# QiminWu/mceik

Measured on AMD Instinct MI355X. Metric: MCMC proposals/sec (FSM eikonal + likelihood), 128³ grid, 1/2/4/8 MI355X, higher is better.
Workload: dtype f32

## Files before the change

mceik_amd/csrc/capi.hip:

```cpp
#include <hip/hip_runtime.h>
#include <float.h>
#include <math.h>
#include <stdint.h>
#include <stdio.h>
#include <stdlib.h>
#include <string.h>
#include <unistd.h>

#include <algorithm>
#include <vector>

#include "../../include/mceik.h"
#include "fsm_common.h"
#include "mcmc_common.h"
#include "fsm_single.h"
#include "rccl_rt.h"
#include "posterior.h"
#include "temper.h"

hipError_t fsm_launch(const FsmLaunch &L, int is_double, int nwaves, hipStream_t st);
hipError_t fsm_zero_words(unsigned *p, int n, hipStream_t st);
int fsm_occupancy(const FsmLaunch &L, int is_double);
size_t fsm_launch_lds_bytes(const FsmLaunch &L, int is_double);
int fsm_launch_kind(const FsmLaunch &L, int is_double);
const char *fsm_launch_name(const FsmLaunch &L, int is_double);
hipError_t fsm_to_brick_f64(const double *src, void *dst, int dst_double, const FsmLaunch &L, int nfield, hipStream_t st);
hipError_t fsm_from_brick_f64(const void *src, int src_double, double *dst, const FsmLaunch &L, int nfield, hipStream_t st);
hipError_t fsm_from_brick_f32(const float *src, float *dst, const FsmLaunch &L, int nfield, hipStream_t st);
hipError_t fsm_to_brick_f32(const float *src, float *dst, const FsmLaunch &L, int nfield, hipStream_t st);
hipError_t mcmc_propose(const McmcDev &D, uint64_t step, hipStream_t st);
hipError_t mcmc_init_loglik(const McmcDev &D, hipStream_t st);
hipError_t mcmc_accept(const McmcDev &D, int keep_slot, hipStream_t st);
hipError_t mcmc_lpt_order(const unsigned long long *clk, int nsolve, int *order, hipStream_t st);
hipError_t l2_gridsearch_f32(int ldgrd, int ngrd, int nev, int iwantOT, float t0use, const int *ev_ptr,
                             const int *obs_row, const float *tc, const float *wt, const float *xnorm,
                             const float *test, float *t0, float *objfn, int negate, hipStream_t st);
size_t relocate_lds_bytes(int nrows, int nobs, int nev);
hipError_t relocate_lds(int ldgrd, int ngrd, int nrows, int nev, int nobs, int iwantOT, float t0use,
                        const int *ev_ptr, const int *obs_row, const float *tc, const float *wt, const float *xnorm,
                        const float *test, float *t0, float *objfn, int negate, hipStream_t st);
hipError_t gridsearch_f90(int is_double, int ldgrd, int ngrd, int nuse, int iwantOT, const int *row,
                          const void *tob, const void *w0, const void *wl, const void *test, void *logpdf,
                          hipStream_t st);
hipError_t l2_gridsearch(int ldgrd, int ngrd, int nuse, int iwantOT, double t0use, const int *use,
                         const double *tc, const double *wt, double xnorm, const double *test,
                         double *t0, double *objfn, hipStream_t st);

#define HIPCHK(x)                                                                      \
    do {                                                                               \
        hipError_t e_ = (x);                                                           \
        if (e_ != hipSuccess) {                                                        \
            fprintf(stderr, "mceik_hip: %s failed: %s (%s:%d)\n", #x,                  \
                    hipGetErrorString(e_), __FILE__, __LINE__);                        \
            return -1;                                                                 \
        }                                                                              \
    } while (0)

static double conv_threshold(double tol, int is_double)
{
    double tolr = is_double ? tol : (double)(float)tol;
    if (!(tolr > 0.0)) return HUGE_VAL;
    int p = is_double ? 53 : 24;
    int k = (int)ceil(log2(tolr)) + p;
    while (ldexp(1.0, k - p) < tolr) k++;
    while (ldexp(1.0, k - 1 - p) >= tolr) k--;
    double T = ldexp(1.0, k);
    double big = is_double ? DBL_MAX : (double)FLT_MAX;
    return T > big ? HUGE_VAL : T;
}

static void fill_launch(FsmLaunch &L, const mceik_fsm_batch *b)
{
    memset(&L, 0, sizeof(L));
    L.nx = b->nx; L.ny = b->ny; L.nz = b->nz;
    fsm_geometry(&L, b->precision == 64 ? 8 : 4);
    L.maxit = b->maxit; L.max_sweeps = b->max_sweeps;
    L.tol = b->tol; L.h = b->h; L.x0 = b->x0; L.y0 = b->y0; L.z0 = b->z0;
    int is_double = b->precision == 64;
    double T = conv_threshold(b->tol, is_double);
    L.conv_thresh = is_double ? (T == HUGE_VAL ? DBL_MAX : T) : (T == HUGE_VAL ? (double)FLT_MAX : T);
    L.nsolve = b->nmodel * b->nstat; L.nstat = b->nstat; L.nsrc = b->nsrc;
    L.src = b->src;
    L.slow_mode = b->slow_mode;
    L.nrx = b->nrx > 0 ? b->nrx : 1; L.nry = b->nry > 0 ? b->nry : 1; L.nrz = b->nrz > 0 ? b->nrz : 1;
    L.ncx = mceik_div_up(L.nx, L.nrx); L.ncy = mceik_div_up(L.ny, L.nry); L.ncz = mceik_div_up(L.nz, L.nrz);
    L.magic_rx = ((1u << 20) + L.nrx - 1) / L.nrx;
    L.magic_ry = ((1u << 20) + L.nry - 1) / L.nry;
    L.magic_rz = ((1u << 20) + L.nrz - 1) / L.nrz;
    L.ev_node = b->ev_node; L.nev = b->nev; L.ttab = b->ttab; L.ev_frac = b->ev_frac;
    L.model_phase = b->slow_mode == 1 ? b->model_phase : nullptr;
    L.skip = b->skip;
    L.solve_count = b->solve_count;
    L.nphase = b->nphase > 0 ? b->nphase : 1;
    {
        auto span = [](int a, int e, int nr) { return e / nr - a / nr + 1; };
        int mx = 0, my = 0, mz = 0;
        for (int t = 0; t < L.ntx; t++) {
            int v = span(t * 8, t * 8 + 7 < L.nx - 1 ? t * 8 + 7 : L.nx - 1, L.nrx); mx = v > mx ? v : mx;
        }
        for (int t = 0; t < L.nty; t++) {
            int v = span(t * 8, t * 8 + 7 < L.ny - 1 ? t * 8 + 7 : L.ny - 1, L.nry); my = v > my ? v : my;
        }
        for (int t = 0; t < L.nzk; t++) {
            int a = t * L.kb * 8, e = a + L.kb * 8 - 1 < L.nz - 1 ? a + L.kb * 8 - 1 : L.nz - 1;
            int v = span(a, e, L.nrz); mz = v > mz ? v : mz;
        }
        L.ccb = mx * my * mz;
        L.cell_cache = b->slow_mode == 1 && L.ccb <= MCEIK_CC_MAX && L.nx < 4096 && L.ny < 4096 && L.nz < 4096;
        if (!L.cell_cache) L.ccb = 0;
    }
    L.fast_sqrt = b->fast_sqrt;
    L.niter = b->niter; L.ierr = b->ierr;
    L.iter_total = b->iter_total;
    L.visit_stats = b->visit_stats;
    L.solve_order = b->solve_order;
    L.solve_clock = b->solve_clock;
    L.max_waves = b->max_waves;
    L.traffic = b->traffic;
    L.step_z = b->step_z;
}

static int g_device_cus = 0;

static int device_cus()
{
    if (g_device_cus == 0) {
        int dev = 0;
        hipDeviceProp_t p;
        if (hipGetDevice(&dev) == hipSuccess && hipGetDeviceProperties(&p, dev) == hipSuccess)
            g_device_cus = p.multiProcessorCount;
        else
            g_device_cus = 256;
    }
    return g_device_cus;
}

static size_t ws_budget_bytes()
{
    static size_t budget = 0;
    if (budget == 0) {
        const char *e = getenv("MCEIK_FSM_WS_GB");
        double gb = e ? atof(e) : 0.0;
        if (gb > 0.0) {
            budget = (size_t)(gb * 1073741824.0);
        } else {
            size_t fr = 0, tot = 0;
            const size_t margin = (size_t)8 << 30;
            if (hipMemGetInfo(&fr, &tot) == hipSuccess && tot) {
                budget = tot / 5 * 4;
                const size_t avail = fr > 2 * margin ? fr - margin : fr / 2;
                if (avail < budget) budget = avail;
            } else {
                budget = (size_t)96 << 30;
            }
        }
    }
    return budget;
}

static int batch_waves(const FsmLaunch &L, int is_double)
{
    int per_cu = fsm_occupancy(L, is_double);
    if (per_cu < 1) per_cu = 1;
    static const int env_cap = [] { const char *e = getenv("MCEIK_WAVES_PER_CU"); return e ? atoi(e) : 0; }();
    if (env_cap > 0 && env_cap < per_cu) per_cu = env_cap;
    long w = (long)per_cu * device_cus();
    if (L.max_waves > 0 && w > L.max_waves) w = L.max_waves;
    if (w > L.nsolve) w = L.nsolve;
    static const bool report = getenv("MCEIK_LAUNCH_REPORT") != nullptr;
    if (report)
        fprintf(stderr, "mceik fsm launch: %d-z steps, %d waves/CU (occupancy), %ld resident waves, %zu B LDS per wave\n",
                fsm_launch_kind(L, is_double), per_cu, w, fsm_launch_lds_bytes(L, is_double));
    return (int)(w < 1 ? 1 : w);
}

static int fsm_batch_waves_uncapped(const mceik_fsm_batch *b)
{
    FsmLaunch L;
    fill_launch(L, b);
    return batch_waves(L, b->precision == 64);
}

struct WsLayout {
    size_t counter, slow, u, u0, zf, total;
    int nwaves;
};

static WsLayout ws_layout(const mceik_fsm_batch *b)
{
    FsmLaunch L;
    fill_launch(L, b);
    int is_double = b->precision == 64;
    size_t es = is_double ? 8 : 4;
    WsLayout w;
    w.nwaves = batch_waves(L, is_double);
    const size_t zfw = fsm_launch_kind(L, is_double) == 16 ? zf_bytes(L, es) : 0;
    {
        const size_t per_wave = 2 * L.field_elems * es + zfw;
        const long cap = (long)(ws_budget_bytes() / (per_wave ? per_wave : 1));
        if (cap >= 1 && w.nwaves > cap) w.nwaves = (int)cap;
    }
    w.counter = 0;
    w.slow = 1024;
    size_t slow_bytes = b->slow_mode == 0 ? (size_t)b->nmodel * L.field_elems * es : 0;
    w.u = w.slow + ((slow_bytes + 255) & ~(size_t)255);
    size_t nu = b->u_out ? (size_t)L.nsolve : (size_t)w.nwaves;
    w.u0 = w.u + nu * L.field_elems * es;
    w.zf = w.u0 + (size_t)w.nwaves * L.field_elems * es;
    w.total = w.zf + (size_t)w.nwaves * zfw;
    return w;
}

extern "C" size_t mceik_fsm_workspace_bytes(const mceik_fsm_batch *b)
{
    return ws_layout(b).total;
}

extern "C" int mceik_fsm_step_z(const mceik_fsm_batch *b)
{
    if (!b) return 0;
    FsmLaunch L;
    fill_launch(L, b);
    return fsm_launch_kind(L, b->precision == 64);
}

extern "C" const char *mceik_fsm_kernel_name(const mceik_fsm_batch *b)
{
    if (!b) return "";
    FsmLaunch L;
    fill_launch(L, b);
    return fsm_launch_name(L, b->precision == 64);
}

extern "C" size_t mceik_fsm_lds_bytes(const mceik_fsm_batch *b)
{
    if (!b) return 0;
    FsmLaunch L;
    fill_launch(L, b);
    return fsm_launch_lds_bytes(L, b->precision == 64);
}

extern "C" double mceik_fsm_bytes_per_node_sweep(const mceik_fsm_batch *b)
{
    double es = b->precision == 64 ? 8.0 : 4.0;
    double s = b->slow_mode == 0 ? es : 4.0 / ((double)b->nrx * b->nry * b->nrz);
    return 2.0 * es + s / (b->nstat > 0 ? b->nstat : 1);
}

#define MCEIK_MC_CHUNK 64
struct McmcExt {
    const void *dev;
    unsigned *sync;
    unsigned spin_limit;
    int step0, nsteps, nburn, keepk, maxs, nkept0;
};

static int fsm_batch_solve_impl(const mceik_fsm_batch *b, void *workspace, size_t workspace_bytes, void *stream,
                                const McmcExt *ext);

extern "C" int mceik_fsm_batch_solve(const mceik_fsm_batch *b, void *workspace, size_t workspace_bytes,
                                     void *stream)
{
    return fsm_batch_solve_impl(b, workspace, workspace_bytes, stream, nullptr);
}

static int fsm_batch_solve_impl(const mceik_fsm_batch *b, void *workspace, size_t workspace_bytes, void *stream,
                                const McmcExt *ext)
{
    if (!b || b->nx < 2 || b->ny < 2 || b->nz < 2 || b->nx > 4096 || b->ny > 4096 || b->nz > 4096 ||
        b->nsrc < 1 ||
        b->nmodel < 1 || b->nstat < 1 || !(b->precision == 32 || b->precision == 64)) {
        fprintf(stderr, "mceik_fsm_batch_solve: invalid batch description\n");
        return 1;
    }
    if (b->slow_mode == 1 && b->precision != 32 && b->precision != 64) return 1;
    WsLayout w = ws_layout(b);
    {
        FsmLaunch G;
        fill_launch(G, b);
        if (G.field_elems * (b->precision == 64 ? 8 : 4) >= (size_t)1 << 31) {
            fprintf(stderr, "mceik_fsm_batch_solve: one travel-time field must stay below 2 GiB\n");
            return 1;
        }
        if (fsm_launch_lds_bytes(G, b->precision == 64) > MCEIK_MAX_LDS) {
            fprintf(stderr, "mceik_fsm_batch_solve: %d x %d x %d z-blocks exceed the LDS block tables\n", G.ntx, G.nty,
                    G.nzk);
            return 1;
        }
        const bool held = fsm_launch_kind(G, b->precision == 64) == 16 || fsm_compact_layout(G, 8);
        const int infl = fsm_launch_kind(G, b->precision == 64) == 16 ? fsm16_geo(G).infl : G.infl;
        if (held && hold_clock_bound(G.nblocks, infl) >= 65536) {
            fprintf(stderr, "mceik_fsm_batch_solve: %d z-blocks overflow the held stream's 16-bit clocks\n", G.nblocks);
            return 1;
        }
    }
    if (!workspace || workspace_bytes < w.total) {
        fprintf(stderr, "mceik_fsm_batch_solve: workspace too small (%zu < %zu)\n", workspace_bytes, w.total);
        return 1;
    }
    if (b->skip && b->u_out) {
        fprintf(stderr, "mceik_fsm_batch_solve: skip and u_out cannot be combined (a skipped solve has no field)\n");
        return 1;
    }
    hipStream_t st = (hipStream_t)stream;
    int is_double = b->precision == 64;
    FsmLaunch L;
    fill_launch(L, b);
    char *ws = (char *)workspace;
    L.counter = (unsigned *)(ws + w.counter);
    HIPCHK(fsm_zero_words(L.counter, 256, st));
    if (b->slow_mode == 0) {
        void *sb = ws + w.slow;
        if (is_double)
            HIPCHK(fsm_to_brick_f64((const double *)b->slow, sb, 1, L, b->nmodel, st));
        else
            HIPCHK(fsm_to_brick_f32((const float *)b->slow, (float *)sb, L, b->nmodel, st));
        L.slow = sb;
    } else {
        L.slow = b->slow;
    }
    L.u = ws + w.u;
    L.u0 = ws + w.u0;
    L.zf = ws + w.zf;
    L.slot_per_solve = b->u_out ? 1 : 0;
    if (ext) {
        if (is_double || fsm_launch_kind(L, 0) != 16 || b->solve_order || b->u_out) return 1;
        L.mc_dev = ext->dev;
        L.mc_sync = ext->sync;
        L.mc_spin_limit = ext->spin_limit;
        L.mc_step0 = ext->step0; L.mc_nsteps = ext->nsteps;
        L.mc_nburn = ext->nburn; L.mc_keepk = ext->keepk; L.mc_maxs = ext->maxs; L.mc_nkept0 = ext->nkept0;
        HIPCHK(fsm_zero_words(ext->sync, MC_SYNC_WORDS(L.nsolve / L.nstat) - 1, st));
    }
    HIPCHK(fsm_launch(L, is_double, w.nwaves, st));
    if (b->u_out) {
        if (is_double) HIPCHK(fsm_from_brick_f64(L.u, 1, (double *)b->u_out, L, L.nsolve, st));
        else HIPCHK(fsm_from_brick_f32((const float *)L.u, (float *)b->u_out, L, L.nsolve, st));
    }
    return 0;
}

static bool is_device_ptr(const void *p)
{
    hipPointerAttribute_t a;
    if (!p || hipPointerGetAttributes(&a, p) != hipSuccess) {
        (void)hipGetLastError();
        return false;
    }
    return a.type == hipMemoryTypeDevice;
}

extern "C" int eikonal3d_batch_solve(int nmodels, int nstations, int nx, int ny, int nz, double h, double x0,
                                     double y0, double z0, int maxit, double tol, const double *src,
                                     const float *slow, float *u, int *niter, int *ierr)
{
    if (nmodels < 1 || nstations < 1 || !src || !slow || !u) return 1;
    const size_t n = (size_t)nx * ny * nz, nsolve = (size_t)nmodels * nstations;
    mceik_fsm_batch b;
    memset(&b, 0, sizeof(b));
    b.nx = nx; b.ny = ny; b.nz = nz; b.h = h; b.x0 = x0; b.y0 = y0; b.z0 = z0;
    b.maxit = maxit; b.tol = tol; b.precision = 32;
    b.nmodel = nmodels; b.nstat = nstations; b.nsrc = 1; b.slow_mode = 0; b.max_sweeps = -1;
    std::vector<void *> tmp;
    auto stage = [&](const void *p, size_t bytes, bool in) -> void * {
        if (is_device_ptr(p)) return const_cast<void *>(p);
        void *d = nullptr;
        if (hipMalloc(&d, bytes) != hipSuccess) return nullptr;
        tmp.push_back(d);
        if (in && hipMemcpy(d, p, bytes, hipMemcpyHostToDevice) != hipSuccess) return nullptr;
        return d;
    };
    int rc = 0;
    void *d_src = stage(src, (size_t)nstations * 4 * sizeof(double), true);
    void *d_slow = stage(slow, (size_t)nmodels * n * sizeof(float), true);
    void *d_u = stage(u, nsolve * n * sizeof(float), false);
    void *d_it = niter ? stage(niter, nsolve * sizeof(int), false) : nullptr;
    void *d_ie = ierr ? stage(ierr, nsolve * sizeof(int), false) : nullptr;
    void *ws = nullptr;
    if (!d_src || !d_slow || !d_u || (niter && !d_it) || (ierr && !d_ie)) rc = -1;
    if (!rc) {
        b.src = (const double *)d_src; b.slow = d_slow; b.u_out = d_u;
        b.niter = (int *)d_it; b.ierr = (int *)d_ie;
        const size_t wsb = mceik_fsm_workspace_bytes(&b);
        if (hipMalloc(&ws, wsb) != hipSuccess) rc = -1;
        else rc = mceik_fsm_batch_solve(&b, ws, wsb, nullptr);
        if (!rc && hipDeviceSynchronize() != hipSuccess) rc = -1;
    }
    if (!rc && d_u != u) rc = hipMemcpy(u, d_u, nsolve * n * sizeof(float), hipMemcpyDeviceToHost) != hipSuccess;
    if (!rc && niter && d_it != niter) rc = hipMemcpy(niter, d_it, nsolve * sizeof(int), hipMemcpyDeviceToHost) != hipSuccess;
    if (!rc && ierr && d_ie != ierr) rc = hipMemcpy(ierr, d_ie, nsolve * sizeof(int), hipMemcpyDeviceToHost) != hipSuccess;
    if (ws) hipFree(ws);
    for (void *p : tmp) hipFree(p);
    return rc;
}

extern "C" int mceik_memcpy(void *dst, const void *src, size_t bytes, int kind)
{
    hipMemcpyKind k = kind == 0 ? hipMemcpyHostToDevice : kind == 1 ? hipMemcpyDeviceToHost : hipMemcpyDeviceToDevice;
    HIPCHK(hipMemcpy(dst, src, bytes, k));
    return 0;
}

struct SingleState {
    int init;
    int nx, ny, nz, maxit_cap, nsrc_cap;
    int is_double;
    SingleLaunch L;
    void *mem;
    double *dense, *src;
    int *ierr_bc;
    int nwaves;
    int bcfail;
    hipStream_t st;
    int iverb, maxit;
    double x0, y0, z0, h, tol;
    BlockDecomp D;
    double *snap;
    unsigned *d_count;
};
static SingleState g_single[3];

static void single_free(SingleState &S)
{
    if (S.snap) hipFree(S.snap);
    if (S.d_count) hipFree(S.d_count);
    if (S.mem) hipFree(S.mem);
    if (S.st) hipStreamDestroy(S.st);
    const SingleState keep = S;
    memset(&S, 0, sizeof(S));
    S.init = keep.init;
    S.iverb = keep.iverb; S.maxit = keep.maxit;
    S.x0 = keep.x0; S.y0 = keep.y0; S.z0 = keep.z0; S.h = keep.h; S.tol = keep.tol;
    S.D = keep.D;
}

static int blocks_buffers(SingleState &S)
{
    const size_t np = (size_t)S.L.nxp * S.L.nyp * S.L.nzp;
    if (!S.snap && hipMalloc(&S.snap, np * 8) != hipSuccess) { S.snap = nullptr; return 1; }
    if (!S.d_count && hipMalloc(&S.d_count, 16) != hipSuccess) { S.d_count = nullptr; return 1; }
    return 0;
}

static int single_alloc(SingleState &S, int is_double, int nx, int ny, int nz, int maxit, int nsrc)
{
    if (S.mem && S.is_double == is_double && S.nx == nx && S.ny == ny && S.nz == nz && maxit <= S.maxit_cap &&
        nsrc <= S.nsrc_cap)
        return 0;
    const int keep = S.init;
    single_free(S);
    S.init = keep;
    if (nx < 1 || ny < 1 || nz < 1 || (long)nx * ny * nz >= (1L << 31)) return 1;
    SingleLaunch &L = S.L;
    L.nx = nx; L.ny = ny; L.nz = nz;
    L.gx = nx; L.gy = ny; L.gz = nz;
    L.nbx = mceik_div_up(nx, 8); L.nby = mceik_div_up(ny, 8); L.nbz = mceik_div_up(nz, 8);
    if (L.nbx > 1024 || L.nby > 1024 || L.nbz > 1024) return 1;
    L.nxp = 8 * L.nbx; L.nyp = 8 * L.nby; L.nzp = 8 * L.nbz;
    L.nb = L.nbx * L.nby * L.nbz;
    if ((size_t)L.nxp * L.nyp * L.nzp * (is_double ? 8 : 4) >= ((size_t)1 << 31)) return 1;
    const int mcap = maxit > 0 ? maxit : 1, scap = nsrc > 0 ? nsrc : 1;
    const size_t es = is_double ? 8 : 4, np = (size_t)L.nxp * L.nyp * L.nzp, n = (size_t)nx * ny * nz;
    auto al = [](size_t v) { return (v + 255) & ~(size_t)255; };
    size_t off[12], o = 0;
    off[0] = o; o += al(np * es);
    off[1] = o; o += al(np * es);
    off[2] = o; o += al(np * es);
    off[3] = o; o += al(np);
    off[4] = o; o += al((size_t)L.nb * 4);
    off[5] = o; o += al((size_t)L.nb * 4);
    off[6] = o; o += al((size_t)(32 + mcap) * 4);
    off[7] = o; o += al((size_t)mcap * 8);
    off[8] = o; o += al((size_t)mcap * 4);
    off[9] = o; o += al(n * 8);
    off[10] = o; o += al((size_t)scap * 32);
    off[11] = o; o += al(16);
    if (hipMalloc(&S.mem, o) != hipSuccess) { S.mem = nullptr; return 1; }
    char *m = (char *)S.mem;
    L.u = m + off[0]; L.u0 = m + off[1]; L.slow = m + off[2]; L.bc = (unsigned char *)(m + off[3]);
    L.border = (const int *)(m + off[4]); L.done = (unsigned *)(m + off[5]); L.ctl = (unsigned *)(m + off[6]);
    L.arrive = (unsigned long long *)(m + off[7]); L.ierr_it = (int *)(m + off[8]);
    S.dense = (double *)(m + off[9]); S.src = (double *)(m + off[10]); S.ierr_bc = (int *)(m + off[11]);
    L.bcerr = S.ierr_bc;
    std::vector<int> ord;
    ord.reserve(L.nb);
    for (int lev = 0; lev <= L.nbx + L.nby + L.nbz - 3; lev++)
        for (int bz = 0; bz < L.nbz; bz++)
            for (int by = 0; by < L.nby; by++) {
                const int bx = lev - bz - by;
                if (bx >= 0 && bx < L.nbx) ord.push_back(bx | (by << 10) | (bz << 20));
            }
    if ((int)ord.size() != L.nb ||
        hipMemcpy((void *)L.border, ord.data(), ord.size() * 4, hipMemcpyHostToDevice) != hipSuccess ||
        hipStreamCreateWithFlags(&S.st, hipStreamNonBlocking) != hipSuccess) {
        single_free(S);
        return 1;
    }
    static const int wpc = [] { const char *e = getenv("MCEIK_SINGLE_WAVES_PER_CU"); return e ? atoi(e) : 2; }();
    int occ = fsm_single_occupancy(is_double);
    S.nwaves = device_cus() * std::max(1, std::min(wpc, occ));
    S.is_double = is_double; S.nx = nx; S.ny = ny; S.nz = nz; S.maxit_cap = mcap; S.nsrc_cap = scap;
    return 0;
}

static int single_solve(SingleState &S, int maxit, int nsrc, double tol, double h, double x0, double y0, double z0,
                        const double *ts, const double *xs, const double *ys, const double *zs, const double *slow,
                        double *u, int *niter_out)
{
    SingleLaunch &L = S.L;
    const size_t n = (size_t)L.nx * L.ny * L.nz;
// ... 1861 lines not shown
```

mceik_amd/csrc/fsm16_kernel.hip:

```cpp
#include <hip/hip_runtime.h>
#include <float.h>
#include <stdint.h>

#include "fsm_common.h"
#include "fsm_device.h"
#include "fsm_hold.h"
#include "fsm_update.h"
#include "mcmc_device.h"

namespace {

__device__ __forceinline__ uint32_t zoff16(int zb)
{
    const uint32_t u = (uint32_t)zb;
    return ((u >> 1) << 13) | ((u & 1u) << 6);
}

#ifdef MCEIK_PHASECLK
#undef TRAF
#undef TRAFU
#define TRAF(S, k, pred, bytes) do { } while (0)
#define TRAFU(S, k, bytes) do { } while (0)
#define PCLK(k)                                                                                         \
    do {                                                                                                \
        const unsigned long long t_ = __builtin_readcyclecounter();                                     \
        if (threadIdx.x == 0) S.scratch[8 + (k)] += (int)(t_ - pclk_t);                                 \
        pclk_t = t_;                                                                                    \
    } while (0)
#else
#define PCLK(k) do { } while (0)
#endif

struct Smem16 {
    int *box;
    float *cc;
    unsigned short *order;
    unsigned short *lastproc;
    unsigned short *lastchg;
    int *ring_e, *ring_b;
    unsigned *ring_base;
    unsigned *fmask;
    int *scratch;
    float *xr;
    unsigned *meta;
    unsigned char *fz;
    unsigned *vbits, *cbits;
};
template <bool FIXED>
__device__ __forceinline__ Smem16 smem16_bind(const FsmLaunch &L, unsigned char *base)
{
    size_t off[MCEIK_SMEM16_ARRAYS];
    if (FIXED) {
        off[8] = F16_CINFO; off[7] = F16_XR; off[1] = F16_CC; off[5] = F16_RING; off[6] = F16_SCRATCH;
        off[3] = F16_LASTPROC; off[4] = F16_LASTCHG; off[2] = F16_ORDER;
        off[9] = F16_ORDER + mceik_align16((size_t)L.ntiles * 2);
        off[10] = off[9] + mceik_align16((size_t)L.ntiles);
        off[0] = off[10] + f16_bitmap_bytes(L);
    } else {
        fsm16_smem_layout(L, off);
    }
    const int nr = fsm16_geo(L).nr;
    Smem16 S;
    S.box = reinterpret_cast<int *>(base + off[0]);
    S.cc = reinterpret_cast<float *>(base + off[1]);
    S.order = reinterpret_cast<unsigned short *>(base + off[2]);
    S.lastproc = reinterpret_cast<unsigned short *>(base + off[3]);
    S.lastchg = reinterpret_cast<unsigned short *>(base + off[4]);
    S.ring_e = reinterpret_cast<int *>(base + off[5]);
    S.ring_b = S.ring_e + (FIXED ? F16_NR : nr);
    S.ring_base = reinterpret_cast<unsigned *>(S.ring_b + (FIXED ? F16_NR : nr));
    S.fmask = S.ring_base + (FIXED ? F16_NR : nr);
    S.fz = base + off[9];
    S.vbits = reinterpret_cast<unsigned *>(base + off[10]);
    S.cbits = S.vbits + (L.nblocks + 31) / 32;
    S.scratch = reinterpret_cast<int *>(base + off[6]);
    S.xr = reinterpret_cast<float *>(base + off[7]);
    S.meta = reinterpret_cast<unsigned *>(base + off[8]);
    return S;
}

#define XROW16(arr, q, row) (((arr) * 4 + (q)) * MCEIK_X16Q + (row) * 4)
typedef float f4v16 __attribute__((ext_vector_type(4)));
__device__ __forceinline__ void lds_w4(float *p, float a, float b, float c, float d)
{
    *reinterpret_cast<f4v16 *>(p) = f4v16{a, b, c, d};
}
__device__ __forceinline__ void lds_r4(const float *p, float &a, float &b, float &c, float &d)
{
    const f4v16 v = *reinterpret_cast<const f4v16 *>(p);
    a = v.x; b = v.y; c = v.z; d = v.w;
}
__device__ __forceinline__ void store_row16(float *x, int arr, int lane, const float (&v)[16])
{
#pragma unroll
    for (int q = 0; q < 4; q++) lds_w4(x + XROW16(arr, q, lane), v[4 * q], v[4 * q + 1], v[4 * q + 2], v[4 * q + 3]);
}
__device__ __forceinline__ void load_row16(const float *x, int arr, int row, float (&v)[16])
{
#pragma unroll
    for (int q = 0; q < 4; q++) lds_r4(x + XROW16(arr, q, row), v[4 * q], v[4 * q + 1], v[4 * q + 2], v[4 * q + 3]);
}
__device__ __forceinline__ void load_half16(const float *x, int arr, int row, int h, float (&v)[8])
{
    lds_r4(x + XROW16(arr, 2 * h, row), v[0], v[1], v[2], v[3]);
    lds_r4(x + XROW16(arr, 2 * h + 1, row), v[4], v[5], v[6], v[7]);
}
__device__ __forceinline__ void halo_stage16(float *x, int lane, const float (&v)[8])
{
    const int j = lane >> 1, h = lane & 1;
    const int arr = (j >> 3) & 1, row = 64 + ((j >> 4) << 3) + (j & 7);
    lds_w4(x + XROW16(arr, 2 * h, row), v[0], v[1], v[2], v[3]);
    lds_w4(x + XROW16(arr, 2 * h + 1, row), v[4], v[5], v[6], v[7]);
}

#define NPASS16 4
#define W1_ZD (1u << 24)

__device__ __forceinline__ void seg_issue(Rsrc r, uint32_t seg, float (&a)[16])
{
    const bool odd = threadIdx.x & 1;
    const uint32_t segp = dpp_swap_pair(seg);
    float t[4];
    bload4(r, odd ? segp + 16u : seg, t);
    a[0] = t[0]; a[1] = t[1]; a[2] = t[2]; a[3] = t[3];
    bload4(r, odd ? segp + 48u : seg + 32u, t);
    a[4] = t[0]; a[5] = t[1]; a[6] = t[2]; a[7] = t[3];
    bload4(r, odd ? seg + 16u : segp, t);
    a[8] = t[0]; a[9] = t[1]; a[10] = t[2]; a[11] = t[3];
    bload4(r, odd ? seg + 48u : segp + 32u, t);
    a[12] = t[0]; a[13] = t[1]; a[14] = t[2]; a[15] = t[3];
}
#define XQE MCEIK_X16Q
__device__ __forceinline__ int pair_row(int arr, int lane)
{
    return (lane & 1) ? XROW16(arr, 1, lane - 1) : XROW16(arr, 0, lane);
}
__device__ __forceinline__ void raw_write(float *x, int pb, const float (&a)[16])
{
    lds_w4(x + pb, a[0], a[1], a[2], a[3]);
    lds_w4(x + pb + 2 * XQE, a[4], a[5], a[6], a[7]);
    lds_w4(x + pb + 4, a[8], a[9], a[10], a[11]);
    lds_w4(x + pb + 2 * XQE + 4, a[12], a[13], a[14], a[15]);
}
__device__ __forceinline__ void raw_read(const float *x, int pb, float (&a)[16])
{
    lds_r4(x + pb, a[0], a[1], a[2], a[3]);
    lds_r4(x + pb + 2 * XQE, a[4], a[5], a[6], a[7]);
    lds_r4(x + pb + 4, a[8], a[9], a[10], a[11]);
    lds_r4(x + pb + 2 * XQE + 4, a[12], a[13], a[14], a[15]);
}
template <int P>
struct Par16 {
    static constexpr int value = P;
};

struct LineLd {
    float a[8];
    int rowl, rowo;
};
__device__ __forceinline__ void line_issue(Rsrc r, uint32_t seg, bool isl, LineLd &q, float (&h)[8])
{
    const int lane = threadIdx.x, par = lane & 1;
    const bool islp = dpp_swap_pair((unsigned)isl) != 0u;
    const uint32_t segp = dpp_swap_pair(seg);
    const uint32_t sl = isl ? seg : (islp ? segp : OOB);
    const uint32_t o = (uint32_t)par * 16u;
    float t[4];
    bload4(r, sl + o, t);
    q.a[0] = t[0]; q.a[1] = t[1]; q.a[2] = t[2]; q.a[3] = t[3];
    bload4(r, sl + o + 32u, t);
    q.a[4] = t[0]; q.a[5] = t[1]; q.a[6] = t[2]; q.a[7] = t[3];
    const uint32_t sh = sl ^ 64u;
    bload4(r, sh + o, t);
    h[0] = t[0]; h[1] = t[1]; h[2] = t[2]; h[3] = t[3];
    bload4(r, sh + o + 32u, t);
    h[4] = t[0]; h[5] = t[1]; h[6] = t[2]; h[7] = t[3];
    q.rowl = isl ? lane : (lane ^ 1);
    q.rowo = lane ^ (q.rowl == lane ? 1 : 0);
}
__device__ __forceinline__ void line_write(float *x, const LineLd &q, const float (&hp)[8])
{
    const int par = threadIdx.x & 1;
    lds_w4(x + XROW16(1, par, q.rowl), q.a[0], q.a[1], q.a[2], q.a[3]);
    lds_w4(x + XROW16(1, par + 2, q.rowl), q.a[4], q.a[5], q.a[6], q.a[7]);
    lds_w4(x + XROW16(1, par, q.rowo), hp[0], hp[1], hp[2], hp[3]);
    lds_w4(x + XROW16(1, par + 2, q.rowo), hp[4], hp[5], hp[6], hp[7]);
}

__device__ __forceinline__ void raw_store(Rsrc r, uint32_t seg, bool chg, const float (&t)[16])
{
    const bool odd = threadIdx.x & 1;
    const uint32_t own = chg ? seg : OOB;
    const uint32_t oth = dpp_swap_pair(own);
    const uint32_t o = odd ? 16u : 0u;
    const uint32_t b01 = (odd ? oth : own) + o, b23 = (odd ? own : oth) + o;
    bstore4(r, b01, t[0], t[1], t[2], t[3]);
    bstore4(r, b01 + 32u, t[4], t[5], t[6], t[7]);
    bstore4(r, b23, t[8], t[9], t[10], t[11]);
    bstore4(r, b23 + 32u, t[12], t[13], t[14], t[15]);
}
__device__ __forceinline__ void store16_plain(Rsrc r, uint32_t off, const float (&v)[16])
{
#pragma unroll
    for (int q = 0; q < 4; q++) bstore4(r, off + 16u * q, v[4 * q], v[4 * q + 1], v[4 * q + 2], v[4 * q + 3]);
}

__device__ __forceinline__ void bload4h(Rsrc r, uint32_t off, float (&v)[4])
{
    f4v a = __builtin_bit_cast(f4v, __builtin_amdgcn_raw_buffer_load_b128(r, off, 0, 0));
    v[0] = a.x; v[1] = a.y; v[2] = a.z; v[3] = a.w;
}
struct BInfo16 {
    uint32_t seg;
    uint32_t zh;
    uint32_t lseg;
    uint32_t w1, w2, w3;
    __device__ __forceinline__ int fl() const { return (int)(w1 & 0xfffu); }
    __device__ __forceinline__ int zb() const { return (int)((w1 >> 12) & 0xffu); }
    __device__ __forceinline__ int ri() const { return (int)((w1 >> 20) & 0xfu); }
    __device__ __forceinline__ int ccb() const { return (int)(w2 << 16) >> 16; }
    __device__ __forceinline__ int clk() const { return (int)(w2 >> 16); }
    __device__ __forceinline__ int bid() const { return (int)(w3 & 0xffffu); }
    __device__ __forceinline__ int bcm() const { return (int)(w3 >> 16); }
};
template <bool RZ>
__device__ __forceinline__ BInfo16 brick_info16(const FsmLaunch &L, const Fsm16Geo &g, int kb, const Smem16 &S,
                                                const Pos &p, int nstream, int lx, int ly, const BcBoxes &bc,
                                                unsigned meta, uint32_t col)
{
    BInfo16 b;
    const int tz = ci_tz(meta);
    const int zb = tz * kb + (RZ ? kb - 1 - p.zbs : p.zbs);
    const bool valid = pos_valid(p, nstream) && (meta & C_BLK) && zb < g.nzb;
    b.seg = valid ? col + zoff16(zb) : OOB;
    b.lseg = pos_valid(p, nstream) && (meta & C_BLK) && (zb & ~1) < g.nzb ? col + zoff16(zb) : OOB;
    const int zu = RZ ? zb * 16 + 16 : zb * 16 - 1;
    b.zh = (valid && (meta & C_ZH) && p.zbs == 0) ? col + zoff16(zu >> 4) + (uint32_t)(zu & 15) * 4u : OOB;
    int fl = valid ? (int)((meta & 0x7f) | F_VALID) : 0;
    if (zb == (RZ ? g.nzb - 1 : 0)) fl |= F_FIRST;
    if (zb == (RZ ? 0 : g.nzb - 1)) fl |= F_LAST;
    const bool zd = valid && p.zbs == kb - 1 && !(fl & F_LAST);
    if (b.zh != OOB) b.zh = zf_boundary<float, RZ>(L, S.ring_b[p.ri], false, lx, ly);
    if (zd) b.zh = zf_boundary<float, RZ>(L, S.ring_b[p.ri], true, lx, ly);
    if ((meta & C_ZH) && p.zbs == 0) fl |= F_ZH;
    bool slow = (fl & C_PART) || ((fl & C_00) && zb == 0) || (valid && zb * 16 + 16 > L.nz);
    unsigned bcm = 0;
    if (__any(fl & C_BC)) {
        const int e = S.ring_e[p.ri];
        const int x = (e & 0xfff) * 8 + lx, y = ((e >> 12) & 0xfff) * 8 + ly;
        unsigned m = 0;
        if (fl & C_BC) {
            for (int k = 0; k < bc.n; k++) {
                const int *q = bc.box + 6 * k;
                if (x >= q[0] && x <= q[1] && y >= q[2] && y <= q[3]) {
                    int lo = q[4] - zb * 16, hi = q[5] - zb * 16;
                    lo = lo < 0 ? 0 : lo; hi = hi > 15 ? 15 : hi;
                    if (lo <= hi) m |= ((2u << hi) - (1u << lo));
                }
            }
        }
        bcm = m;
        slow |= m != 0;
    }
    if (slow) fl |= F_SLOW;
    const int ccb = ci_ccb(meta) + zb * 4;
    b.w1 = (uint32_t)fl | ((uint32_t)(valid ? zb : 0) << 12) | ((uint32_t)p.ri << 20) | (zd ? W1_ZD : 0u);
    b.w2 = ((uint32_t)ccb & 0xffffu) | ((uint32_t)p.sp << 16);
    b.w3 = ((uint32_t)S.ring_b[p.ri] & 0xffffu) | (bcm << 16);
    return b;
}
template <bool RZ>
__device__ __forceinline__ uint32_t halo_offset16(const Fsm16Geo &g, int kb, const Pos &pe, int nstream, int half,
                                                  unsigned meta, uint32_t col, unsigned hbit, uint32_t hdelta)
{
    const int zb = ci_tz(meta) * kb + (RZ ? kb - 1 - pe.zbs : pe.zbs);
    const bool valid = pos_valid(pe, nstream) && (meta & C_BLK) && zb < g.nzb;
    const uint32_t base = col + ((meta & hbit) ? 0u : hdelta);
    return valid ? base + zoff16(zb) + (uint32_t)half * 32u : OOB;
}

#define LW_G(p) (9 + 5 * (p))
#define LW_CCB 19
template <bool RZ>
__device__ __forceinline__ unsigned lean_word(const FsmLaunch &L, const Fsm16Geo &g, const ColTile &ct, int tz, int ri,
                                              int u0flag, int zh)
{
    int cz0, nczb;
    block_zcells(L, L.kb, tz, cz0, nczb);
    const int m = ct.fl | C_BLK | (u0flag ? C_U0 : 0) | (zh ? C_ZH : 0);
    const int zb0 = 2 * tz + (RZ ? 1 : 0);
    unsigned w = (unsigned)m & 0x1ffu;
#pragma unroll
    for (int p = 0; p < 2; p++) {
        const int zb = RZ ? zb0 - p : zb0 + p;
        unsigned gp = zb < g.nzb ? 16u : 0u;
        if (zb == (RZ ? g.nzb - 1 : 0)) gp |= 1u;
        if (zb == (RZ ? 0 : g.nzb - 1)) gp |= 2u;
        if ((m & C_PART) || ((m & C_00) && zb == 0) || zb * 16 + 16 > L.nz) gp |= 4u;
        if (p == 0 && (m & C_ZH)) gp |= 8u;
        w |= gp << LW_G(p);
    }
    const int ccb0 = ri * L.ccb + ct.cl * nczb - cz0 + zb0 * 4;
    return w | ((unsigned)ccb0 << LW_CCB);
}
template <bool RZ>
__device__ __forceinline__ BInfo16 brick_info_lean(const FsmLaunch &L, const Smem16 &S, const Pos &p, int nstream,
                                                   int lx, int ly, const BcBoxes &bc, unsigned w, uint32_t base)
{
    BInfo16 b;
    const int ph = p.zbs;
    const unsigned gp = (w >> (ph ? LW_G(1) : LW_G(0))) & 31u;
    const bool pv = pos_valid(p, nstream);
    const bool valid = pv && (gp & 16u);
    const uint32_t off = base + ((uint32_t)(ph ^ (RZ ? 1 : 0)) << 6);
    b.seg = valid ? off : OOB;
    b.lseg = pv && (w & ((16u << LW_G(0)) | (16u << LW_G(1)))) ? off : OOB;
    b.zh = valid && (gp & 8u) ? off + (RZ ? 8192u - 64u : 124u - 8192u) : OOB;
    const bool zd = valid && ph == 1 && !(gp & 2u);
    if (b.zh != OOB) b.zh = zf_boundary<float, RZ>(L, S.ring_b[p.ri], false, lx, ly);
    if (zd) b.zh = zf_boundary<float, RZ>(L, S.ring_b[p.ri], true, lx, ly);
    int fl = valid ? (int)((w & 0x7fu) | F_VALID | ((gp & 15u) << 8)) : 0;
    unsigned bcm = 0;
    if (__any(fl & C_BC)) {
        const int e = S.ring_e[p.ri];
        const int zb = 2 * ((e >> 24) & 0xff) + (RZ ? 1 - ph : ph);
        const int x = (e & 0xfff) * 8 + lx, y = ((e >> 12) & 0xfff) * 8 + ly;
        if (fl & C_BC) {
            for (int k = 0; k < bc.n; k++) {
                const int *q = bc.box + 6 * k;
                if (x >= q[0] && x <= q[1] && y >= q[2] && y <= q[3]) {
                    int lo = q[4] - zb * 16, hi = q[5] - zb * 16;
                    lo = lo < 0 ? 0 : lo; hi = hi > 15 ? 15 : hi;
                    if (lo <= hi) bcm |= ((2u << hi) - (1u << lo));
                }
            }
        }
        if (bcm) fl |= F_SLOW;
    }
    const int ccb = (int)(w >> LW_CCB) + (RZ ? -4 * ph : 4 * ph);
    b.w1 = (uint32_t)fl | ((uint32_t)ph << 12) | ((uint32_t)p.ri << 20) | (zd ? W1_ZD : 0u);
    b.w2 = ((uint32_t)ccb & 0xffffu) | ((uint32_t)p.sp << 16);
    b.w3 = ((uint32_t)S.ring_b[p.ri] & 0xffffu) | (bcm << 16);
    return b;
}
template <bool RZ>
__device__ __forceinline__ uint32_t halo_offset_lean(const Pos &pe, int nstream, int half, unsigned me, uint32_t base,
                                                     unsigned hbit, uint32_t hdelta)
{
    const int ph = pe.zbs;
    const bool valid = pos_valid(pe, nstream) && ((me >> (ph ? LW_G(1) : LW_G(0))) & 16u);
    const uint32_t o = base + ((me & hbit) ? 0u : hdelta) + ((uint32_t)(ph ^ (RZ ? 1 : 0)) << 6) + (uint32_t)half * 32u;
    return valid ? o : OOB;
}
template <bool RZ>
__device__ __forceinline__ uint32_t halo_line_lean(const Pos &pe, int nstream, unsigned me, uint32_t base,
                                                   unsigned hbit, uint32_t hdelta)
{
    const bool valid = pos_valid(pe, nstream) && (me & ((16u << LW_G(0)) | (16u << LW_G(1))));
    return valid ? base + ((me & hbit) ? 0u : hdelta) : OOB;
}
__device__ __forceinline__ unsigned dpp_swap_quad_half(unsigned v)
{
    return (unsigned)__builtin_amdgcn_mov_dpp((int)v, 0x4E, 0xf, 0xf, false);
}
template <bool RZ, bool LEAN>
__device__ __forceinline__ BInfo16 brick_info_any(const FsmLaunch &L, const Fsm16Geo &g, int kb, const Smem16 &S,
                                                  const Pos &p, int nstream, int lx, int ly, const BcBoxes &bc,
                                                  unsigned meta, uint32_t col)
{
    if (LEAN) return brick_info_lean<RZ>(L, S, p, nstream, lx, ly, bc, meta, col);
    return brick_info16<RZ>(L, g, kb, S, p, nstream, lx, ly, bc, meta, col);
}
template <bool RZ, bool LEAN>
__device__ __forceinline__ uint32_t halo_offset_any(const Fsm16Geo &g, int kb, const Pos &pe, int nstream, int half,
                                                    unsigned meta, uint32_t col, unsigned hbit, uint32_t hdelta)
{
    if (LEAN) return halo_offset_lean<RZ>(pe, nstream, half, meta, col, hbit, hdelta);
    return halo_offset16<RZ>(g, kb, pe, nstream, half, meta, col, hbit, hdelta);
}

__device__ __forceinline__ void build_order16(const FsmLaunch &L, unsigned short *order)
{
    for (int id = threadIdx.x; id < L.ntiles; id += 64) {
        const int txs = id % L.ntx, tys = id / L.ntx, dg = txs + tys;
        int rank = 0;
        for (int e = 0; e < dg; e++)
            rank += min(e, L.nty - 1) - max(0, e - L.ntx + 1) + 1;
        rank += tys - max(0, dg - L.ntx + 1);
        order[rank] = (unsigned short)(txs | (tys << 8));
    }
}


__device__ __forceinline__ HoldLds<unsigned short> hold_lds16(const Smem16 &S)
{
    HoldLds<unsigned short> H;
    H.order = S.order; H.fz = S.fz; H.lastproc = S.lastproc; H.need = S.lastchg; H.fmask = S.fmask;
    H.ring_e = S.ring_e; H.vbits = S.vbits; H.cbits = S.cbits;
    return H;
}


template <bool RZ, bool LEAN>
__device__ __forceinline__ void admit16(const FsmLaunch &L, const Fsm16Geo &g, const Smem16 &S, const BcBoxes &bc,
                                        int entry, int zh, int u0flag, int ri, int C, int lx, int ly, int lxs,
                                        int lys, int rx, int ry, ColTile &ct)
{
    unsigned meta = 0;
    int bid = 0, nbv = 0;
    uint32_t base = 0;
    if (entry >= 0) {
        const int tz = (entry >> 24) & 0xff, tx = entry & 0xfff, ty = (entry >> 12) & 0xfff;
        bid = tz * L.ntiles + tx + ty * L.ntx;
        nbv = min(L.kb, L.nzb - tz * L.kb);
        if ((entry & 0xffffff) != ct.tile) column_tile<float>(L, bc, entry, lx, ly, lxs, lys, rx, ry, ct);
        meta = LEAN ? lean_word<RZ>(L, g, ct, tz, ri, u0flag, zh) : column_word(L, L.kb, ct, tz, ri, u0flag, zh);
        base = (uint32_t)(ty * L.ntx + tx) * tile_bytes<float>(L) + (LEAN ? (uint32_t)tz << 13 : 0u);
    }
    const int nact = L.visit_stats && entry >= 0 ? __builtin_popcountll(__ballot(ct.fl & C_ACT)) : 0;
    asm volatile("" ::: "memory");
    S.meta[ri * 64 + threadIdx.x] = meta;
    if (threadIdx.x == 0) {
        if (entry >= 0) {
            S.lastproc[bid] = (unsigned short)C;
            S.vbits[bid >> 5] |= 1u << (bid & 31);
            if (L.visit_stats) {
                S.scratch[0] += nbv;
                S.scratch[1] += nbv * nact;
            }
        }
        S.ring_e[ri] = entry;
        S.ring_b[ri] = bid;
        S.ring_base[ri] = base;
    }
    asm volatile("" ::: "memory");
}


template <bool RZ, bool GENERIC, bool LEAN, bool NC = true>
__device__ __forceinline__ void brick16(const FsmLaunch &L, const Smem16 &S, const BInfo16 &b0, float (&v)[16],
                                        float zprev0, float znext, int lx, int ly, int rx, int ry, bool &changed,
                                        bool &nc, int &ierr_last, bool &c0, bool &c15)
{
    const int lane = threadIdx.x;
    const float T = (float)L.conv_thresh;
    const int fl = b0.fl();
    bool xp = true, xn = true, yp = true, yn = true, act = true;
    int zbg = 0;
    if (GENERIC) {
        const int e = S.ring_e[b0.ri()];
        zbg = LEAN ? 2 * ((e >> 24) & 0xff) + (RZ ? 1 - b0.zb() : b0.zb()) : b0.zb();
        const int x = (e & 0xfff) * 8 + lx, y = ((e >> 12) & 0xfff) * 8 + ly;
        const bool xlo = x > 0, xhi = x < L.nx - 1, ylo = y > 0, yhi = y < L.ny - 1;
        xp = rx ? xhi : xlo; xn = rx ? xlo : xhi; yp = ry ? yhi : ylo; yn = ry ? ylo : yhi;
        act = (fl & C_ACT) != 0;
    }
    const bool first = (fl & F_FIRST) != 0, last = (fl & F_LAST) != 0;
    const int lxs = lane & 7, lys = lane >> 3;
    const int rxm = lxs > 0 ? lane - 1 : 64 + lys, rym = lys > 0 ? lane - 8 : 72 + lxs;
    const int rxp = lxs < 7 ? lane + 1 : 64 + lys, ryp = lys < 7 ? lane + 8 : 72 + lxs;
    float fc = 0.f, ffc = 0.f, ff2c = 0.f, ff3c = 0.f;
#pragma unroll
    for (int hh = 0; hh < NPASS16; hh++) {
        constexpr int PZ = 16 / NPASS16;
        const int h = RZ ? NPASS16 - 1 - hh : hh;
        float xm[PZ], xq[PZ], ym[PZ], yq[PZ];
        lds_r4(S.xr + XROW16(0, h, rxm), xm[0], xm[1], xm[2], xm[3]);
        lds_r4(S.xr + XROW16(0, h, rym), ym[0], ym[1], ym[2], ym[3]);
        lds_r4(S.xr + XROW16(1, h, rxp), xq[0], xq[1], xq[2], xq[3]);
        lds_r4(S.xr + XROW16(1, h, ryp), yq[0], yq[1], yq[2], yq[3]);
#pragma unroll
        for (int jj = 0; jj < PZ; jj++) {
            const int j = hh * PZ + jj;
            const int pj = RZ ? 15 - j : j;
            const int ph = pj % PZ;
            const int pprev = RZ ? pj + 1 : pj - 1, pnext = RZ ? pj - 1 : pj + 1;
            const float self = v[pj];
            if (!GENERIC) {
                if ((j & 3) == 0) {
                    fc = S.cc[b0.ccb() + (pj >> 2)];
                    ffc = fc * fc;
                    ff2c = ffc + ffc;
                    ff3c = 3.0f * ffc;
                }
            }
            float xup = xm[ph], xdn = xq[ph], yup = ym[ph], ydn = yq[ph];
            float zup, zdn;
            if (GENERIC) {
                xup = xp ? xup : self; xdn = xn ? xdn : self; yup = yp ? yup : self; ydn = yn ? ydn : self;
                const int zabs = zbg * 16 + pj;
                const bool zp_ex = RZ ? (zabs < L.nz - 1) : (zabs > 0);
                const bool zn_ex = RZ ? (zabs > 0) : (zabs < L.nz - 1);
                zup = zp_ex ? (j > 0 ? v[pprev] : zprev0) : self;
                zdn = zn_ex ? (j < 15 ? v[pnext] : znext) : self;
            } else {
                zup = j > 0 ? v[pprev] : (first ? self : zprev0);
                zdn = j < 15 ? v[pnext] : (last ? self : znext);
            }
            const float ux = fmin_(xup, xdn), uy = fmin_(yup, ydn), uz = fmin_(zup, zdn);
            float nv;
            if (GENERIC) {
                const int zabs = zbg * 16 + pj;
                const int zc_ = zabs < L.nz ? zabs : L.nz - 1;
                const float f = S.cc[b0.ccb() - zbg * 4 + (zc_ >> 2)];
                int e;
                const float ub = godunov_bl<true>(ux, uy, uz, f, e);
                const bool upd = act && zabs < L.nz && !((b0.bcm() >> pj) & 1);
                nv = upd ? fmin_(self, ub) : self;
                if ((fl & C_00) && zabs == 0) ierr_last = upd ? e : 0;
            } else {
                nv = fmin_(self, godunov_v<true>(ux, uy, uz, fc, ffc, ff2c, ff3c));
            }
            const bool dec = nv < self;
            if (NC) nc |= dec && self >= T;
            changed |= dec;
            if (pj == 0) c0 = dec;
            if (pj == 15) c15 = dec;
            v[pj] = nv;
        }
    }
}

template <bool RZ, int KB16, int CCR>
__device__ __forceinline__ int sweep16(const FsmLaunch &L, const Fsm16Geo &g, Rsrc ur, Rsrc u0r, Rsrc sr, Rsrc zfr,
                                       const BcBoxes &bc, const Smem16 &S, int rx, int ry, int clock0, bool &notconv,
                                       int &ierr_last, unsigned &nchg, unsigned &nsteps)
{
    const Rsrc zr_ = zfr;
#ifdef MCEIK_PHASECLK
    unsigned long long pclk_t = __builtin_readcyclecounter();
#endif
    const int lane = threadIdx.x, lxs = lane & 7, lys = lane >> 3, d = lxs + lys;
    const int lx = rx ? 7 - lxs : lxs, ly = ry ? 7 - lys : lys;
    const float UN = FLT_MAX;
    const int kb = KB16 > 0 ? KB16 : g.kb;
    const int nr = KB16 > 0 ? F16_NR : g.nr;
    const uint32_t lanecol = (uint32_t)colpos(lx, ly) * 128u;

    const int hj = lane >> 1, hh = lane & 1, he = halo_edge_lane(hj), hd = (he & 7) + (he >> 3);
    const unsigned hbit = hj < 16 ? C_XOWN : C_YOWN;
    const uint32_t hdelta = halo_delta(L, tile_bytes<float>(L), hj, he, rx, ry);
    const int hlx = rx ? 7 - (he & 7) : (he & 7), hly = ry ? 7 - (he >> 3) : (he >> 3);
    const uint32_t hcol = (uint32_t)colpos(hlx, hly) * 128u;

    const HoldLds<unsigned short> H = hold_lds16(S);
    const unsigned xyface = HOLD_OWN | (lx == 0 ? 2u : 0u) | (lx == 7 ? 4u : 0u) | (ly == 0 ? 8u : 0u) |
                            (ly == 7 ? 16u : 0u);
    hold_norm(L, H);
    if (lane == 0) { S.scratch[4] = 0; S.scratch[5] = -1; }
    clock0 = 64;
    auto decide_any = [&](int pos, int ri, int &zh, int &u0) __attribute__((always_inline)) -> int {
        const HoldSt hs = hold_state(S.scratch + 4);
        const int q = pos - g.infl;
        if (q >= 0) hold_settle(L, H, q % nr, clock0 + q);
        return hold_decide<RZ>(L, H, S.scratch + 4, hs, clock0 + pos, rx, ry, ri == 0 ? nr - 1 : ri - 1, g.infl,
                               g.vis, zh, u0);
    };
    constexpr bool FL = KB16 == 2;
    constexpr bool LEAN = KB16 == 2;
    float v[16], qa[16], hs[2][8];
    LineLd lq;
    float hps[2][8];
    float (&hq)[8] = hs[0];
    constexpr bool HFL = FL && LEAN;
    const int hr = lane & 3, hpi = (lane >> 4) & 1, hcme = (lane >> 1) & 1;
    const int hj0 = (lane >> 1) & ~1;
    const int hst = XROW16((hj0 >> 3) & 1, hr, 64 + ((hj0 >> 4) << 3) + (hj0 & 7));
    float hA[2][4], hB[2][4], hBs[4];
    float (&hn)[8] = hs[1];
    float (&hp)[8] = hps[0];
    float zc, zn, zq;
    float ccv[CCR];
    int ccsize = 0;
    ColTile ct;
    ct.tile = -1;
    constexpr int AH = MCEIK_AHEAD16;
    int ndecided = 0, nstream = 0x7fffffff, dri = 0;
    for (int pos = 0; pos <= (AH - 1) / kb; pos++) {
        int zh, u0;
        const int e = decide_any(pos, dri, zh, u0);
        if (e == -2) {
            if (pos == 0) return 0;
            nstream = pos;
            break;
        }
        admit16<RZ, LEAN>(L, g, S, bc, e, zh, u0, dri, clock0 + pos, lx, ly, lxs, lys, rx, ry, ct);
        if (e >= 0) {
            cc_issue<CCR>(L, L.kb, sr, e, ccv, ccsize);
            TRAFU(S, 5, ccsize * 4);
            cc_write<float, CCR>(L, S.cc, dri, ccv, ccsize, (float)L.h);
        }
        ndecided = pos + 1;
        if (++dri == nr) dri = 0;
    }
    asm volatile("" ::: "memory");
    Pos p3, pe;
    pos_init(p3, -d, kb, nr);
    BInfo16 b0 = brick_info_any<RZ, LEAN>(L, g, kb, S, p3, nstream, lx, ly, bc, S.meta[p3.ri * 64 + lane],
                                  S.ring_base[p3.ri] + lanecol);
    const int pbr = pair_row(0, lane), pbn = pair_row(1, lane);
    {
        float t[16];
        seg_issue(ur, b0.seg, t);
        raw_write(S.xr, pbn, t);
        load_row16(S.xr, 1, lane, v);
    }
    pos_init(pe, -hd, kb, nr);
    {
        const uint32_t ho = halo_offset_any<RZ, LEAN>(g, kb, pe, nstream, hh, S.meta[pe.ri * 64 + he],
                                              S.ring_base[pe.ri] + hcol, hbit, hdelta);
        bload4h(ur, ho, *reinterpret_cast<float (*)[4]>(&hq[0]));
        bload4h(ur, ho + 16u, *reinterpret_cast<float (*)[4]>(&hq[4]));
        TRAF(S, 1, ho != OOB, 32);
    }
    zc = bload1(zr_, b0.zh, 0.0f);
    TRAF(S, 0, b0.seg != OOB, 64);
    TRAF(S, 2, b0.zh != OOB, 4);
    pos_adv(p3, kb, nr);
    BInfo16 b1 = brick_info_any<RZ, LEAN>(L, g, kb, S, p3, nstream, lx, ly, bc, S.meta[p3.ri * 64 + lane],
                                  S.ring_base[p3.ri] + lanecol);
    {
        float t[16];
        seg_issue(ur, b1.seg, t);
        raw_write(S.xr, pbn, t);
    }
    if (FL) {
        Pos pn = p3;
        pos_adv(pn, kb, nr);
        const bool nl = pn.vb >= 0 && pn.zbs == 1;
        const uint32_t sn = nl ? brick_info_any<RZ, LEAN>(L, g, kb, S, pn, nstream, lx, ly, bc, S.meta[pn.ri * 64 + lane],
                                                  S.ring_base[pn.ri] + lanecol).seg
                               : OOB;
        const bool nlp = dpp_swap_pair((unsigned)nl) != 0u;
        const uint32_t snp = dpp_swap_pair(sn);
        const uint32_t s0 = (nl ? sn : (nlp ? snp : OOB)) + (uint32_t)(lane & 1) * 16u;
        float t[4];
        bload4(ur, s0, t);
        hp[0] = t[0]; hp[1] = t[1]; hp[2] = t[2]; hp[3] = t[3];
        bload4(ur, s0 + 32u, t);
        hp[4] = t[0]; hp[5] = t[1]; hp[6] = t[2]; hp[7] = t[3];
#pragma unroll
        for (int i = 0; i < 8; i++) asm volatile("" : "+v"(hp[i]));
    }
    pos_adv(pe, kb, nr);
    if (HFL) {
        const uint32_t lo = halo_line_lean<RZ>(pe, nstream, S.meta[pe.ri * 64 + he], S.ring_base[pe.ri] + hcol, hbit,
                                               hdelta);
        const uint32_t lp = dpp_swap_quad_half(lo);
        const uint32_t l1 = hcme == (hpi ^ 1) ? lo : lp, l0 = hcme == hpi ? lo : lp;
        const uint32_t qo = 16u * (uint32_t)hr, oa = (RZ ? 64u : 0u) + qo, ob = (RZ ? 0u : 64u) + qo;
        bload4h(ur, l1 + oa, hA[1]);
        bload4h(ur, l0 + ob, hB[0]);
        bload4h(ur, l1 + ob, hB[1]);
        TRAF(S, 1, l1 != OOB, 32);
    } else {
        const uint32_t ho = halo_offset_any<RZ, LEAN>(g, kb, pe, nstream, hh, S.meta[pe.ri * 64 + he],
                                              S.ring_base[pe.ri] + hcol, hbit, hdelta);
        bload4h(ur, ho, *reinterpret_cast<float (*)[4]>(&hn[0]));
        bload4h(ur, ho + 16u, *reinterpret_cast<float (*)[4]>(&hn[4]));
        TRAF(S, 1, ho != OOB, 32);
    }
    zn = bload1(zr_, b1.zh, 0.0f);
    TRAF(S, 0, b1.seg != OOB, 64);
    TRAF(S, 2, b1.zh != OOB, 4);
    {
        float un[16];
#pragma unroll
        for (int i = 0; i < 16; i++) un[i] = UN;
        store_row16(S.xr, 0, lane, un);
    }
    halo_stage16(S.xr, lane, hq);
    float zprev = UN;
    if (HFL) {
#pragma unroll
        for (int i = 0; i < 4; i++) asm volatile("" : "+v"(hA[1][i]), "+v"(hB[0][i]), "+v"(hB[1][i]));
    } else {
#pragma unroll
        for (int i = 0; i < 8; i++) hs[0][i] = hs[1][i];
#pragma unroll
        for (int i = 0; i < 8; i++) asm volatile("" : "+v"(hs[0][i]));
    }
#pragma unroll
    for (int i = 0; i < 16; i++) asm volatile("" : "+v"(v[i]));
    asm volatile("" : "+v"(zc), "+v"(zn));
    asm volatile("" ::: "memory");

    int ph = AH % kb;
    int cc_pend = -1;
    int B = 0;
    bool ccfill = false;
    int ccri = 0;
    auto decide_step = [&]() __attribute__((always_inline)) {
        ccfill = false;
        ccri = 0;
        if (ph == 0 && nstream == 0x7fffffff) {
            const int pos = ndecided;
            int zh, u0;
            const int e = decide_any(pos, dri, zh, u0);
            PCLK(4);
            if (e == -2) {
                nstream = pos;
            } else {
                admit16<RZ, LEAN>(L, g, S, bc, e, zh, u0, dri, clock0 + pos, lx, ly, lxs, lys, rx, ry, ct);
                if (e >= 0) {
                    cc_issue<CCR>(L, L.kb, sr, e, ccv, ccsize);
                    TRAFU(S, 5, ccsize * 4);
                    ccfill = true;
                    ccri = dri;
                }
                ndecided = pos + 1;
                if (++dri == nr) dri = 0;
            }
        }
    };
    auto more = [&]() __attribute__((always_inline)) -> bool {
        return !(nstream != 0x7fffffff && B >= nstream * kb + 14);
    };
    auto step = [&](auto par) __attribute__((always_inline)) -> bool {
        constexpr int P = FL ? decltype(par)::value : 0;
        float (&hcur)[8] = hs[P];
        float (&hnew)[8] = hs[1 - P];
        float (&hpcur)[8] = hps[P];
        float (&hpnew)[8] = hps[1 - P];
        pos_adv(p3, kb, nr);
        pos_adv(pe, kb, nr);
        const unsigned m3 = S.meta[p3.ri * 64 + lane], me = S.meta[pe.ri * 64 + he];
        const uint32_t c3 = S.ring_base[p3.ri] + lanecol, ce = S.ring_base[pe.ri] + hcol;
        __builtin_amdgcn_sched_barrier(0);
        const BInfo16 b3 = brick_info_any<RZ, LEAN>(L, g, kb, S, p3, nstream, lx, ly, bc, m3, c3);
        if (FL)
            line_issue(ur, b3.lseg, p3.vb >= 0 && p3.zbs == 0, lq, hpnew);
        else
            seg_issue(ur, b3.seg, qa);
        zq = __any(b3.zh != OOB) ? bload1(zr_, b3.zh, 0.0f) : 0.0f;
        if (HFL) {
            const uint32_t lo = halo_line_lean<RZ>(pe, nstream, me, ce, hbit, hdelta);
            const uint32_t lp = dpp_swap_quad_half(lo);
            const uint32_t sl = hcme == (hpi ^ P) ? lo : lp;
            const uint32_t qo = 16u * (uint32_t)hr;
#pragma unroll
            for (int i = 0; i < 4; i++) hBs[i] = hB[P][i];
            bload4h(ur, sl + (RZ ? 64u : 0u) + qo, hA[P]);
            bload4h(ur, sl + (RZ ? 0u : 64u) + qo, hB[P]);
            TRAF(S, 1, sl != OOB, 32);
            TRAF(S, 0, b3.seg != OOB, 64);
            TRAF(S, 2, b3.zh != OOB, 4);
        } else {
            const uint32_t ho = halo_offset_any<RZ, LEAN>(g, kb, pe, nstream, hh, me, ce, hbit, hdelta);
            bload4h(ur, ho, *reinterpret_cast<float (*)[4]>(&hnew[0]));
            bload4h(ur, ho + 16u, *reinterpret_cast<float (*)[4]>(&hnew[4]));
            TRAF(S, 1, ho != OOB, 32);
            TRAF(S, 0, b3.seg != OOB, 64);
            TRAF(S, 2, b3.zh != OOB, 4);
        }
        PCLK(0);
        __builtin_amdgcn_s_setprio(0);
        const bool wnc = !__any(notconv);
        if (wnc && __any(b0.fl() & C_U0)) {
            unsigned m = __builtin_bit_cast(unsigned, v[0]);
#pragma unroll
            for (int i = 1; i < 16; i++) m = min(m, __builtin_bit_cast(unsigned, v[i]));
            const bool st0 = __builtin_bit_cast(float, m) < (float)L.conv_thresh && (b0.fl() & C_U0);
            if (__any(st0)) store16_plain(u0r, st0 ? b0.seg : OOB, v);
            TRAF(S, 4, st0, 64);
        }
        float znext = S.xr[XROW16(1, RZ ? 3 : 0, lane) + (RZ ? 3 : 0)];
        const unsigned fmk = S.fmask[b0.ri()];
        if ((b0.w1 & W1_ZD) && !(fmk & HOLD_CONT)) znext = zc;
        const float zp0 = (b0.fl() & F_ZH) ? zc : zprev;
        PCLK(1);
        bool changed = false, nc = false, c0 = false, c15 = false;
        if (__any(b0.fl() & F_SLOW))
            brick16<RZ, true, LEAN>(L, S, b0, v, zp0, znext, lx, ly, rx, ry, changed, nc, ierr_last, c0, c15);
        else if (wnc)
            brick16<RZ, false, LEAN>(L, S, b0, v, zp0, znext, lx, ly, rx, ry, changed, nc, ierr_last, c0, c15);
        else
            brick16<RZ, false, LEAN, false>(L, S, b0, v, zp0, znext, lx, ly, rx, ry, changed, nc, ierr_last, c0, c15);
        const bool val = (b0.fl() & F_VALID) != 0;
        changed = changed && val;
        notconv |= nc && val;
        nchg += changed ? 2u : 0u;
        PCLK(2);
        __builtin_amdgcn_s_setprio(2);

        if (cc_pend >= 0) cc_write<float, CCR>(L, S.cc, cc_pend, ccv, ccsize, (float)L.h);
        cc_pend = ccfill ? ccri : -1;
        float nn[16];
        if (FL) {
#pragma unroll
            for (int i = 0; i < 8; i++) asm volatile("" : "+v"(lq.a[i]), "+v"(hpnew[i]));
        } else {
#pragma unroll
            for (int i = 0; i < 16; i++) nn[i] = qa[i];
        }
        if (HFL) {
            const int lc = hpi ^ P;
            lds_w4(S.xr + hst + 4 * (1 - lc), hA[1 - P][0], hA[1 - P][1], hA[1 - P][2], hA[1 - P][3]);
            lds_w4(S.xr + hst + 4 * lc, hBs[0], hBs[1], hBs[2], hBs[3]);
        } else {
            halo_stage16(S.xr, lane, hcur);
        }
        zc = zn; zn = zq;
        if (!FL) {
#pragma unroll
            for (int i = 0; i < 16; i++) asm volatile("" : "+v"(nn[i]));
        }
        if (!FL) {
#pragma unroll
            for (int i = 0; i < 8; i++) hcur[i] = hnew[i];
        }
        if (HFL) {
#pragma unroll
            for (int i = 0; i < 4; i++) asm volatile("" : "+v"(hA[P][i]), "+v"(hB[P][i]));
        } else {
            asm volatile("" : "+v"(hnew[0]), "+v"(hnew[1]), "+v"(hnew[2]), "+v"(hnew[3]), "+v"(hnew[4]),
                         "+v"(hnew[5]), "+v"(hnew[6]), "+v"(hnew[7]));
        }
        asm volatile("" : "+v"(zn));
        asm volatile("" ::: "memory");
        store_row16(S.xr, 0, lane, v);
        zprev = v[RZ ? 0 : 15];
        if (__any(changed)) {
            float t[16];
            raw_read(S.xr, pbr, t);
            raw_store(ur, b0.seg, changed, t);
        }
        TRAF(S, 3, changed, 64);
        {
            const int zr = LEAN ? (b0.zb() ^ (RZ ? 1 : 0)) : b0.zb() % kb;
            const bool zlo = changed && zr == 0 && c0, zhi = changed && zr == kb - 1 && c15;
            if (changed) atomicOr(&S.fmask[b0.ri()], xyface | (zlo ? HOLD_ZLO : 0u) | (zhi ? HOLD_ZHI : 0u));
            if (__any(zlo || zhi)) {
                bstore1(zfr, zlo ? zf_off<float>(b0.bid(), 0, lx, ly) : OOB, v[0]);
                bstore1(zfr, zhi ? zf_off<float>(b0.bid(), 1, lx, ly) : OOB, v[15]);
            }
        }
        load_row16(S.xr, 1, lane, v);
        if (FL) {
            line_write(S.xr, lq, hpcur);
        } else {
            raw_write(S.xr, pbn, nn);
        }
        asm volatile("" ::: "memory");
        b0 = b1;
        b1 = b3;
        if (++ph == kb) ph = 0;
        B++;
        PCLK(3);
        decide_step();
        PCLK(5);
        return more();
    };
    decide_step();
    PCLK(6);
    if (more()) {
        if (FL) {
            do {
                if (!step(Par16<0>())) break;
            } while (step(Par16<1>()));
        } else {
            do {
            } while (step(Par16<0>()));
        }
    }
    __builtin_amdgcn_s_setprio(0);
    nsteps += (unsigned)B;
    for (int q = max(0, nstream - g.infl + 1); q < nstream; q++) hold_settle(L, H, q % nr, clock0 + q);
    PCLK(6);
    return nstream;
}

__device__ __forceinline__ void verify16(const FsmLaunch &L, Rsrc ur, Rsrc u0r, const Smem16 &S, bool &notconv)
{
    const int lane = threadIdx.x, lx = lane & 7, ly = lane >> 3;
    const float T = (float)L.conv_thresh, tolr = (float)L.tol;
    for (int base = 0; base < L.nblocks; base += 64) {
        const int k = base + lane;
        const bool flag = k < L.nblocks && ((S.cbits[k >> 5] >> (k & 31)) & 1u) != 0;
        unsigned long long m = __ballot(flag);
        while (m) {
            const int bid = base + __builtin_ctzll(m);
            m &= m - 1;
            const int tz = bid / L.ntiles, id = bid - tz * L.ntiles;
            const int tx = id % L.ntx, ty = id / L.ntx;
            const int x = tx * 8 + lx, y = ty * 8 + ly;
            const int zend = min(tz * L.kb + L.kb, L.nzb);
            for (int zb = tz * L.kb; zb < zend; zb++) {
                const uint32_t seg = (uint32_t)id * tile_bytes<float>(L) + zoff_bytes<float>(zb) +
                                     (uint32_t)colpos(lx, ly) * 128u;
                float u[8], v0[8];
                bload8(ur, seg, u);
                bload8(u0r, seg, v0);
                TRAF(S, 6, x < L.nx && y < L.ny, 64);
#pragma unroll
                for (int i = 0; i < 8; i++) {
                    float dl = v0[i] - u[i];
                    dl = dl < 0.0f ? -dl : dl;
                    if (x < L.nx && y < L.ny && zb * 8 + i < L.nz && u[i] < T && !(dl < tolr)) notconv = true;
                }
            }
        }
    }
}

struct McQueue {
    unsigned xcc;
    int cur;
};
__device__ __forceinline__ unsigned mc_group_tickets(const FsmLaunch &L, int g, int &clo)
{
    const int nch = L.nsolve / L.nstat;
    clo = (int)((long long)nch * g / 8);
    const int chi = (int)((long long)nch * (g + 1) / 8);
    return (unsigned)(chi - clo) * (unsigned)L.nstat;
}
__device__ __forceinline__ void mc_l1_invalidate()
{
    asm volatile("buffer_inv sc1\n\ts_waitcnt vmcnt(0)" ::: "memory");
}
__device__ __forceinline__ void mc_stores_done()
{
    asm volatile("s_waitcnt vmcnt(0)" ::: "memory");
}
__device__ __forceinline__ bool mc_next(const FsmLaunch &L, McQueue &q, int &solve, int &k)
{
    const int lane = threadIdx.x;
    unsigned *owner = L.mc_sync, *tick = L.mc_sync + 8;
    int *ready = reinterpret_cast<int *>(L.mc_sync + 8 + 8 * 32);
    for (;;) {
        if (q.cur >= 0) {
            int clo;
            const unsigned gs = mc_group_tickets(L, q.cur, clo), tot = gs * (unsigned)L.mc_nsteps;
            unsigned t = 0;
            if (lane == 0) t = atomicAdd(tick + 32 * q.cur, 1u);
            t = __builtin_amdgcn_readfirstlane(__shfl(t, 0, 64));
            if (t < tot) {
                k = (int)(t / gs);
                solve = clo * L.nstat + (int)(t - (unsigned)k * gs);
                const int c = solve / L.nstat;
                unsigned broken = 0;
                if (lane == 0) {
                    for (unsigned it = 0; atomicAdd(ready + c, 0) < k; it++) {
                        if (it >= L.mc_spin_limit) {
                            atomicExch(L.mc_sync + MC_SYNC_WORDS(L.nsolve / L.nstat) - 1, 1u);
                            broken = 1;
                            break;
                        }
                        __builtin_amdgcn_s_sleep(32);
                    }
                }
                broken = __builtin_amdgcn_readfirstlane(__shfl(broken, 0, 64));
                if (broken) return false;
                __builtin_amdgcn_wave_barrier();
                mc_l1_invalidate();
                return true;
            }
            q.cur = -1;
        }
        int found = -1;
        for (int j = 0; j < 8 && found < 0; j++) {
            const int g = (int)((q.xcc - 1u + (unsigned)j) & 7u);
            unsigned own = 0, left = 0;
            if (lane == 0) {
                own = atomicCAS(owner + g, 0u, q.xcc);
                if (own == 0u) own = q.xcc;
                int clo;
                const unsigned tot = mc_group_tickets(L, g, clo) * (unsigned)L.mc_nsteps;
                left = own == q.xcc && atomicAdd(tick + 32 * g, 0u) < tot ? 1u : 0u;
            }
            left = __builtin_amdgcn_readfirstlane(__shfl(left, 0, 64));
            if (left) found = g;
        }
        if (found < 0) return false;
        q.cur = found;
    }
}
__device__ __forceinline__ int mc_keep_slot(const FsmLaunch &L, long long gs)
{
    if (!L.mc_maxs || gs < L.mc_nburn || (gs - L.mc_nburn) % L.mc_keepk) return -1;
    auto nk = [&](long long x) -> long long {
        return x <= L.mc_nburn ? 0 : (x - L.mc_nburn + L.mc_keepk - 1) / L.mc_keepk;
    };
    return (int)((L.mc_nkept0 + nk(gs) - nk(L.mc_step0)) % L.mc_maxs);
}
__device__ __forceinline__ void mc_finish(const FsmLaunch &L, int solve, int k)
{
    const int lane = threadIdx.x;
    const int nch = L.nsolve / L.nstat, c = solve / L.nstat;
    int *ready = reinterpret_cast<int *>(L.mc_sync + 8 + 8 * 32);
    unsigned *done = L.mc_sync + 8 + 8 * 32 + nch;
    mc_stores_done();
    unsigned old = 0;
    if (lane == 0) old = atomicAdd(done + c, 1u);
    old = __builtin_amdgcn_readfirstlane(__shfl(old, 0, 64));
    if (old + 1u != (unsigned)(k + 1) * (unsigned)L.nstat) return;
    mc_l1_invalidate();
    const McmcDev &D = *reinterpret_cast<const McmcDev *>(L.mc_dev);
    const long long gstep = (long long)L.mc_step0 + k;
    const int keep_slot = mc_keep_slot(L, gstep);
    const int inp = mcmcd::ldv(&D.prop_inprior[c]), ph = mcmcd::ldv(&D.prop_phase[c]);
    double ln = 0.0;
    if (inp) {
        for (int e0 = 0; e0 < D.nev; e0 += 64) {
            const int e = e0 + lane, n = min(64, D.nev - e0);
            const double obj = e < D.nev ? mcmcd::event_obj(D, c, ph, e) : 0.0;
            for (int i = 0; i < n; i++) ln = ln - __shfl(obj, i, 64);
        }
    }
    int acc = 0;
    if (lane == 0) acc = mcmcd::chain_accept(D, c, ln, keep_slot);
    acc = __builtin_amdgcn_readfirstlane(__shfl(acc, 0, 64));
    if (acc && D.nphase > 1) mcmcd::chain_copy_tables(D, c, ph, lane, 64);
    if (keep_slot >= 0) {
        const int cell = mcmcd::ldv(&D.prop_cell[c]), pv = mcmcd::ldv(&D.prop_v[c]);
        int *dst = D.keep_v + ((size_t)keep_slot * D.keep_stride + c) * D.ncm;
        const int *src = D.v + (size_t)c * D.ncm;
        for (int j = lane; j < D.ncm; j += 64) dst[j] = (acc && j == cell) ? pv : mcmcd::ldv(src + j);
    }
    if (k + 1 < L.mc_nsteps && lane == 0) mcmcd::chain_propose(D, c, (uint64_t)(gstep + 1));
    mc_stores_done();
    if (lane == 0) atomicExch(ready + c, k + 1);
}

template <int KB16, int CCR, bool MC>
__device__ __forceinline__ void fsm16_body(const FsmLaunch &L)
{
    extern __shared__ __attribute__((aligned(16))) unsigned char smem[];
    const Smem16 S = smem16_bind<KB16 == 2>(L, smem);
    const Fsm16Geo g = fsm16_geo(L);
    const int lane = threadIdx.x;
    const uint32_t fbytes = (uint32_t)(L.field_elems * 4);
    build_order16(L, S.order);
    int pass = 0;
    McQueue mq;
    mq.cur = -1;
    mq.xcc = 1u;
    if (MC) {
        unsigned x;
        asm volatile("s_getreg_b32 %0, hwreg(HW_REG_XCC_ID)" : "=s"(x));
        mq.xcc = (x & 0xfu) + 1u;
    }
    for (;;) {
        int snext, mk = 0;
        if (MC) {
            if (!mc_next(L, mq, snext, mk)) break;
        } else {
            snext = next_solve(L, pass);
            if (snext < 0) break;
        }
        const unsigned solve = (unsigned)snext;
        if (L.solve_clock && lane == 0) L.solve_clock[2 * (size_t)solve] = __builtin_amdgcn_s_memrealtime();
        const int model = (int)solve / L.nstat, station = (int)solve - model * L.nstat;
        const size_t slot = L.slot_per_solve ? solve : blockIdx.x;
        float *u = reinterpret_cast<float *>(L.u) + slot * L.field_elems;
        float *u0 = reinterpret_cast<float *>(L.u0) + (size_t)blockIdx.x * L.field_elems;
        const size_t ncell = (size_t)L.ncx * L.ncy * L.ncz;
        const int phase = L.model_phase ? (MC ? mcmcd::ldv(L.model_phase + model) : L.model_phase[model])
                                        : fsm_plain_phase(L, model);
        if (L.skip && L.skip[phase * L.nstat + station]) {
            skip_solve<float>(L, solve);
            if (MC) mc_finish(L, (int)solve, mk);
            __builtin_amdgcn_s_waitcnt(0);
            __builtin_amdgcn_fence(__ATOMIC_SEQ_CST, "workgroup");
            continue;
        }
        const size_t sentry = !L.model_phase ? (size_t)model : (size_t)model * L.nphase + phase;
        const void *slow_model = reinterpret_cast<const float *>(L.slow) + sentry * ncell;
        const Rsrc ur = make_rsrc(u, fbytes), u0r = make_rsrc(u0, fbytes),
                   sr = make_rsrc(slow_model, (uint32_t)(ncell * 4));
        const size_t zfb = zf_bytes(L, 4);
        const Rsrc zfr = make_rsrc(reinterpret_cast<char *>(L.zf) + (size_t)blockIdx.x * zfb, (uint32_t)zfb);
        if (lane == 0) { S.scratch[0] = 0; S.scratch[1] = 0; S.scratch[2] = 0; S.scratch[3] = 0; }
#ifdef MCEIK_TRAFFIC
        if (lane == 0)
            for (int k = 0; k < MCEIK_TRAFFIC_N; k++) S.scratch[8 + k] = 0;
#endif
        unsigned nchg = 0, nsteps = 0;
        BcBoxes bc;
        bc.box = S.box;
        const bool ok = init_field<float, 1>(L, u, ur, slow_model, L.src + (size_t)station * L.nsrc * 4, bc);
        hold_solve_start(L, hold_lds16(S), bc, g.nr);
        zf_init<float>(L, zfr, u, bc);
        asm volatile("" ::: "memory");
        int iters = 0, ierr_last = 0;
        if (ok) {
            int sweeps_left = L.max_sweeps < 0 ? 0x7fffffff : L.max_sweeps;
            for (int it = 0; it < L.maxit && sweeps_left > 0; it++) {
                bool notconv = false;
                hold_iter_start(L, hold_lds16(S));
                int clock = 64;
                for (int sw = 0; sw < 8 && sweeps_left > 0; sw++, sweeps_left--) {
                    const int rx = sw & 1, ry = (sw >> 1) & 1;
                    if (sw & 4)
                        clock += g.infl + sweep16<true, KB16, CCR>(L, g, ur, u0r, sr, zfr, bc, S, rx, ry, clock, notconv,
                                                              ierr_last, nchg, nsteps);
                    else
                        clock += g.infl + sweep16<false, KB16, CCR>(L, g, ur, u0r, sr, zfr, bc, S, rx, ry, clock, notconv,
                                                               ierr_last, nchg, nsteps);
                    __builtin_amdgcn_s_waitcnt(0);
                    __builtin_amdgcn_fence(__ATOMIC_SEQ_CST, "workgroup");
                    TRAF_FLUSH(L, S);
                }
                iters = it + 1;
                if (sweeps_left > 0 || L.max_sweeps < 0) {
                    if (!__any(notconv)) verify16(L, ur, u0r, S, notconv);
                    if (!__any(notconv)) break;
                }
            }
        }
        int ierr = ierr_last;
        for (int o = 32; o > 0; o >>= 1) ierr = max(ierr, __shfl_xor(ierr, o, 64));
        if (!ok) ierr = 1;
        if (L.visit_stats) {
            for (int o = 32; o > 0; o >>= 1) nchg += __shfl_xor(nchg, o, 64);
            asm volatile("" ::: "memory");
            if (lane == 0) {
                atomicAdd(L.visit_stats, (unsigned long long)(unsigned)S.scratch[0]);
                atomicAdd(L.visit_stats + 1, (unsigned long long)(unsigned)S.scratch[1]);
                atomicAdd(L.visit_stats + 2, (unsigned long long)nchg);
                atomicAdd(L.visit_stats + 3, (unsigned long long)nsteps);
            }
        }
        if (lane == 0) {
            if (L.solve_clock) L.solve_clock[2 * (size_t)solve + 1] = __builtin_amdgcn_s_memrealtime();
            if (L.iter_total) atomicAdd(L.iter_total, (unsigned long long)iters);
            if (L.solve_count) atomicAdd(L.solve_count, 1ull);
            if (L.niter) L.niter[solve] = iters;
            if (L.ierr) L.ierr[solve] = ierr;
        }
        TRAFU(S, 7, (unsigned)(L.field_elems * 4) + (L.ttab ? (unsigned)L.nev * (4u + 64u) : 0u));
        TRAF_FLUSH(L, S);
        if (L.ttab) {
            for (int e = lane; e < L.nev; e += 64) L.ttab[(size_t)solve * L.nev + e] = event_time<float>(L, u, e);
        }
        if (MC) mc_finish(L, (int)solve, mk);
        __builtin_amdgcn_s_waitcnt(0);
        __builtin_amdgcn_fence(__ATOMIC_SEQ_CST, "workgroup");
    }
}

#define FSM16_WPE __attribute__((amdgpu_waves_per_eu(2, 2)))
template <int KB16, int CCR, bool MC>
__global__ __launch_bounds__(64) FSM16_WPE void fsm16_solve_kernel(FsmLaunch L)
{
    fsm16_body<KB16, CCR, MC>(L);
}

}

hipError_t fsm16_launch(const FsmLaunch &L, int nwaves, hipStream_t st)
{
    if (!fsm16_eligible(L, 4)) return hipErrorInvalidValue;
    const size_t lds = fsm16_lds_bytes(L);
    const bool mc = L.mc_dev != nullptr;
    if (fsm16_fixed_layout(L)) {
        if (mc) hipLaunchKernelGGL((fsm16_solve_kernel<2, 1, true>), dim3(nwaves), dim3(64), lds, st, L);
        else hipLaunchKernelGGL((fsm16_solve_kernel<2, 1, false>), dim3(nwaves), dim3(64), lds, st, L);
    } else if (L.ccb <= 64) {
        if (mc) hipLaunchKernelGGL((fsm16_solve_kernel<0, 1, true>), dim3(nwaves), dim3(64), lds, st, L);
        else hipLaunchKernelGGL((fsm16_solve_kernel<0, 1, false>), dim3(nwaves), dim3(64), lds, st, L);
    } else {
        if (mc) hipLaunchKernelGGL((fsm16_solve_kernel<0, 4, true>), dim3(nwaves), dim3(64), lds, st, L);
        else hipLaunchKernelGGL((fsm16_solve_kernel<0, 4, false>), dim3(nwaves), dim3(64), lds, st, L);
    }
    return hipGetLastError();
}

int fsm16_occupancy(const FsmLaunch &L)
{
    int nb = 0;
    const size_t lds = fsm16_lds_bytes(L);
    hipError_t e;
    if (fsm16_fixed_layout(L))
        e = hipOccupancyMaxActiveBlocksPerMultiprocessor(&nb, fsm16_solve_kernel<2, 1, false>, 64, lds);
    else if (L.ccb <= 64)
        e = hipOccupancyMaxActiveBlocksPerMultiprocessor(&nb, fsm16_solve_kernel<0, 1, false>, 64, lds);
    else
        e = hipOccupancyMaxActiveBlocksPerMultiprocessor(&nb, fsm16_solve_kernel<0, 4, false>, 64, lds);
    return e == hipSuccess ? nb : 1;
}
```

mceik_amd/csrc/fsm_common.h:

```cpp
#pragma once
#include <stddef.h>
#include <stdint.h>
#include <hip/hip_runtime.h>

#define MCEIK_TILE 8
#define MCEIK_BRICK 512
#define MCEIK_KB 4
#define MCEIK_MAX_BLOCKS 1024
#define MCEIK_AHEAD 2

struct FsmLaunch {
    int nx, ny, nz;
    int ntx, nty, nzb, ntiles;
    int kb, nzk, nblocks, nr;
    int infl, vis;
    int ccb;
    int maxit, max_sweeps;
    double tol, h, x0, y0, z0;
    double conv_thresh;
    int nsolve, nstat, nsrc;
    const double *src;
    int slow_mode;
    const void *slow;
    int ncx, ncy, ncz, nrx, nry, nrz;
    unsigned magic_rx, magic_ry, magic_rz;
    int nzq;
    size_t field_elems;
    void *u;
    void *u0;
    void *zf;
    int slot_per_solve;
    const int *ev_node;
    int nev;
    float *ttab;
    int *niter;
    int *ierr;
    int cell_cache;
    int fast_sqrt;
    unsigned *counter;
    unsigned long long *iter_total;
    unsigned long long *visit_stats;
    const int *solve_order;
    unsigned long long *solve_clock;
    int max_waves;
    unsigned long long *traffic;
    int step_z;
    const float *ev_frac;
    const int *model_phase;
    int nphase;
    const unsigned char *skip;
    unsigned long long *solve_count;
    const void *mc_dev;
    unsigned *mc_sync;
    unsigned mc_spin_limit;
    int mc_step0, mc_nsteps;
    int mc_nburn, mc_keepk, mc_maxs, mc_nkept0;
};
#define MC_SYNC_WORDS(nchains) (8 + 8 * 32 + 2 * (nchains) + 1)

static inline __host__ __device__ int fsm_plain_phase(const FsmLaunch &L, int m)
{
    return L.nphase > 1 ? m % L.nphase : 0;
}

static inline __host__ __device__ size_t fsm_slow_entry(const FsmLaunch &L, int m)
{
    return L.model_phase ? (size_t)m * L.nphase + L.model_phase[m] : (size_t)m;
}

static inline __host__ __device__ int mceik_div_up(int a, int b) { return (a + b - 1) / b; }
static inline __host__ __device__ size_t zf_bytes(const FsmLaunch &L, size_t es) { return (size_t)L.nblocks * 128 * es; }

#if defined(MCEIK_TRAFFIC)
#define MCEIK_SCRATCH_BYTES 64
#else
#define MCEIK_SCRATCH_BYTES 32
#endif
#define MCEIK_TRAFFIC_N 8

#define MCEIK_CC_MAX 256
#define MCEIK_F64_HOLD (2 * 64 * 16)
#define MCEIK_SMEM_ARRAYS 14
#define MCEIK_XROWS 80
static inline __host__ __device__ size_t mceik_align16(size_t v) { return (v + 15) & ~(size_t)15; }
#define FSMF_NR (2 + (16 + MCEIK_KB - 1) / MCEIK_KB)
#define FSMF_CINFO 0
#define FSMF_XR (FSMF_CINFO + FSMF_NR * 64 * 8)
#define FSMF_XN (FSMF_XR + 2 * MCEIK_XROWS * 16)
#define FSMF_CC (FSMF_XN + 2 * MCEIK_XROWS * 16)
#define FSMF_RING (FSMF_CC + FSMF_NR * 64 * 4)
#define FSMF_SCRATCH (FSMF_RING + 64)
#define FSMF_LASTPROC (FSMF_SCRATCH + MCEIK_SCRATCH_BYTES)
#define FSMF_LASTCHG (FSMF_LASTPROC + MCEIK_MAX_BLOCKS * 4)
#define FSMF_ORDER (FSMF_LASTCHG + MCEIK_MAX_BLOCKS * 4)
static inline __host__ __device__ bool fsm_fixed_layout(const FsmLaunch &L, size_t es)
{
    return es == 4 && L.slow_mode != 0 && L.cell_cache && L.fast_sqrt && L.nrz == 4 && L.ccb <= 64 &&
           L.kb == MCEIK_KB && L.nr == FSMF_NR && L.nblocks <= MCEIK_MAX_BLOCKS;
}
static inline __host__ __device__ bool fsm_compact_layout(const FsmLaunch &L, size_t es)
{
    return es == 8 && L.slow_mode != 0 && L.cell_cache && L.nrz == 4 && L.ccb <= 64 && L.kb == MCEIK_KB &&
           L.nblocks <= MCEIK_MAX_BLOCKS;
}
static inline __host__ __device__ size_t fsm_smem_layout(const FsmLaunch &L, size_t es, size_t *off)
{
    if (fsm_fixed_layout(L, es)) {
        off[11] = FSMF_CINFO; off[9] = FSMF_XR; off[10] = FSMF_XN; off[1] = FSMF_CC;
        off[6] = FSMF_RING; off[7] = FSMF_SCRATCH; off[3] = FSMF_LASTPROC; off[4] = FSMF_LASTCHG;
        off[5] = FSMF_ORDER; off[2] = FSMF_ORDER; off[8] = FSMF_ORDER;
        off[0] = FSMF_ORDER + mceik_align16((size_t)L.ntiles * 4);
        off[12] = off[13] = off[0];
        return off[0] + mceik_align16((size_t)(L.nsrc > 0 ? L.nsrc : 1) * 6 * 4);
    }
    const bool cached = L.slow_mode != 0 && L.cell_cache;
    const size_t nt = (size_t)L.ntiles, nb = (size_t)L.nblocks, nr = (size_t)L.nr;
    size_t o = 0;
    off[0] = o; o += mceik_align16((size_t)(L.nsrc > 0 ? L.nsrc : 1) * 6 * 4);
    off[1] = o; o += cached ? mceik_align16(nr * L.ccb * 4) : 0;
    const bool cmp = fsm_compact_layout(L, es);
    off[2] = o; o += mceik_align16(nt * 4);
    off[3] = o; o += mceik_align16(nb * (cmp ? 2 : 4));
    off[4] = o; o += mceik_align16(nb * (cmp ? 2 : 4));
    off[5] = o;
    off[6] = o; o += mceik_align16(nr * (cmp ? 16 : 8));
    off[12] = o; o += cmp ? mceik_align16(nt) : 0;
    off[13] = o; o += cmp ? mceik_align16((nb + 31) / 32 * 4 * 2) : 0;
    off[7] = o; o += MCEIK_SCRATCH_BYTES;
    off[8] = o; o += cached ? 0 : 512 * es;
    off[9] = o; o += 2 * MCEIK_XROWS * 4 * es;
    off[10] = o; o += 2 * MCEIK_XROWS * 4 * es + (es == 8 ? MCEIK_F64_HOLD : 0);
    off[11] = o; o += nr * 64 * (cmp ? 4 : 8);
    return o;
}
static inline size_t fsm_lds_bytes(const FsmLaunch &L, size_t es)
{
    size_t off[MCEIK_SMEM_ARRAYS];
    return fsm_smem_layout(L, es, off);
}
#define MCEIK_MAX_LDS (64 * 1024)

#define MCEIK_AHEAD16 2
struct Fsm16Geo {
    int nzb, kb, nr, infl, vis;
};
static inline __host__ __device__ Fsm16Geo fsm16_geo(const FsmLaunch &L)
{
    Fsm16Geo g;
    g.nzb = mceik_div_up(L.nz, 16);
    g.kb = L.kb / 2;
    g.infl = 1 + mceik_div_up(14 + MCEIK_AHEAD16, g.kb);
    g.vis = mceik_div_up(12, g.kb);
    g.nr = 1 + mceik_div_up(15 + MCEIK_AHEAD16, g.kb);
    return g;
}
static inline __host__ __device__ bool fsm16_eligible(const FsmLaunch &L, size_t es)
{
    return es == 4 && L.slow_mode != 0 && L.cell_cache && L.fast_sqrt && L.nrz == 4 && L.ccb <= MCEIK_CC_MAX &&
           L.kb >= 4 && (L.kb & 1) == 0 && L.nblocks <= MCEIK_MAX_BLOCKS && L.ntx <= 256 && L.nty <= 256;
}
#define MCEIK_SMEM16_ARRAYS 11
#define MCEIK_X16PAD 4
#define MCEIK_X16Q (MCEIK_XROWS * 4 + MCEIK_X16PAD)
#define F16_NR (1 + (15 + MCEIK_AHEAD16 + 1) / 2)
#define F16_CINFO 0
#define F16_XR (F16_CINFO + F16_NR * 64 * 4)
#define F16_CC (F16_XR + 2 * 4 * MCEIK_X16Q * 4)
#define F16_RING (F16_CC + F16_NR * 32 * 4)
#define F16_SCRATCH (F16_RING + 176)
#define F16_LASTPROC (F16_SCRATCH + MCEIK_SCRATCH_BYTES)
#define F16_LASTCHG (F16_LASTPROC + MCEIK_MAX_BLOCKS * 2)
#define F16_ORDER (F16_LASTCHG + MCEIK_MAX_BLOCKS * 2)
static inline __host__ __device__ bool fsm16_fixed_layout(const FsmLaunch &L)
{
    return fsm16_eligible(L, 4) && L.kb == 4 && L.ccb <= 32 && fsm16_geo(L).nr == F16_NR;
}
static inline __host__ __device__ size_t f16_bitmap_bytes(const FsmLaunch &L)
{
    return mceik_align16((size_t)((L.nblocks + 31) / 32) * 4 * 2);
}
static inline __host__ __device__ size_t fsm16_smem_layout(const FsmLaunch &L, size_t *off)
{
    const size_t nbox = mceik_align16((size_t)(L.nsrc > 0 ? L.nsrc : 1) * 6 * 4);
    if (fsm16_fixed_layout(L)) {
        off[8] = F16_CINFO; off[7] = F16_XR; off[1] = F16_CC; off[5] = F16_RING; off[6] = F16_SCRATCH;
        off[3] = F16_LASTPROC; off[4] = F16_LASTCHG; off[2] = F16_ORDER;
        off[9] = F16_ORDER + mceik_align16((size_t)L.ntiles * 2);
        off[10] = off[9] + mceik_align16((size_t)L.ntiles);
        off[0] = off[10] + f16_bitmap_bytes(L);
        return off[0] + nbox;
    }
    const Fsm16Geo g = fsm16_geo(L);
    const size_t nr = (size_t)g.nr, nb = (size_t)L.nblocks;
    size_t o = 0;
    off[0] = o; o += nbox;
    off[1] = o; o += mceik_align16(nr * L.ccb * 4);
    off[2] = o; o += mceik_align16((size_t)L.ntiles * 2);
    off[3] = o; o += mceik_align16(nb * 2);
    off[4] = o; o += mceik_align16(nb * 2);
    off[9] = o; o += mceik_align16((size_t)L.ntiles);
    off[10] = o; o += f16_bitmap_bytes(L);
    off[5] = o; o += mceik_align16(nr * 16);
    off[6] = o; o += MCEIK_SCRATCH_BYTES;
    off[7] = o; o += 2 * 4 * MCEIK_X16Q * 4;
    off[8] = o; o += nr * 64 * 4;
    return o;
}
static inline size_t fsm16_lds_bytes(const FsmLaunch &L)
{
    size_t off[MCEIK_SMEM16_ARRAYS];
    return fsm16_smem_layout(L, off);
}

static inline __host__ __device__ constexpr int hold_clock_bound(int nblocks, int infl)
{
    return nblocks * (1 + infl) + 64;
}
static_assert(hold_clock_bound(MCEIK_MAX_BLOCKS, 1 + (14 + MCEIK_AHEAD16 + 1) / 2) < 65536,
              "16-bit held-stream clocks: MCEIK_MAX_BLOCKS / MCEIK_AHEAD16 too large");
static_assert(hold_clock_bound(MCEIK_MAX_BLOCKS, 1 + (14 + MCEIK_AHEAD + MCEIK_KB - 1) / MCEIK_KB) < 65536,
              "16-bit held-stream clocks: MCEIK_MAX_BLOCKS / MCEIK_AHEAD too large");

static inline void fsm_geometry(FsmLaunch *L, int es)
{
    L->ntx = mceik_div_up(L->nx, MCEIK_TILE);
    L->nty = mceik_div_up(L->ny, MCEIK_TILE);
    L->nzb = mceik_div_up(L->nz, MCEIK_TILE);
    L->ntiles = L->ntx * L->nty;
    int kb = L->nzb < MCEIK_KB ? L->nzb : MCEIK_KB;
    while (kb < L->nzb && ((long)L->ntiles * mceik_div_up(L->nzb, kb) > MCEIK_MAX_BLOCKS || mceik_div_up(L->nzb, kb) > 128))
        kb *= 2;
    if (kb > L->nzb) kb = L->nzb;
    L->kb = kb;
    L->nzk = mceik_div_up(L->nzb, kb);
    L->nblocks = L->ntiles * L->nzk;
    L->infl = 1 + mceik_div_up(14 + MCEIK_AHEAD, kb);
    L->vis = mceik_div_up(12, kb);
    L->nr = 2 + mceik_div_up(16, kb);
    const int bpl = 16 / es;
    L->nzq = mceik_div_up(L->nzb, bpl);
    L->field_elems = (size_t)L->ntiles * L->nzq * 64 * (128 / es);
}
```

mceik_amd/csrc/fsm_device.h:

```cpp
#pragma once
#include <hip/hip_runtime.h>
#include <float.h>
#include <stdint.h>

#include "fsm_common.h"
#include "fsm_update.h"

namespace {

#define OOB 0x80000000u
typedef __amdgpu_buffer_rsrc_t Rsrc;

__device__ __forceinline__ Rsrc make_rsrc(const void *p, uint32_t bytes)
{
    return __builtin_amdgcn_make_buffer_rsrc(const_cast<void *>(p), 0, bytes, 0x00020000);
}

typedef float f4v __attribute__((ext_vector_type(4)));
typedef double d2v __attribute__((ext_vector_type(2)));
typedef unsigned u4v __attribute__((ext_vector_type(4)));
typedef unsigned u2v __attribute__((ext_vector_type(2)));

__device__ __forceinline__ void bload8(Rsrc r, uint32_t off, float (&v)[8])
{
    f4v a = __builtin_bit_cast(f4v, __builtin_amdgcn_raw_buffer_load_b128(r, off, 0, 0));
    f4v b = __builtin_bit_cast(f4v, __builtin_amdgcn_raw_buffer_load_b128(r, off + 16, 0, 0));
    v[0] = a.x; v[1] = a.y; v[2] = a.z; v[3] = a.w; v[4] = b.x; v[5] = b.y; v[6] = b.z; v[7] = b.w;
}
__device__ __forceinline__ void bstore8(Rsrc r, uint32_t off, const float (&v)[8])
{
    f4v a = {v[0], v[1], v[2], v[3]}, b = {v[4], v[5], v[6], v[7]};
    __builtin_amdgcn_raw_buffer_store_b128(__builtin_bit_cast(u4v, a), r, off, 0, 0);
    __builtin_amdgcn_raw_buffer_store_b128(__builtin_bit_cast(u4v, b), r, off + 16, 0, 0);
}
__device__ __forceinline__ void bload8(Rsrc r, uint32_t off, double (&v)[8])
{
#pragma unroll
    for (int k = 0; k < 4; k++) {
        d2v a = __builtin_bit_cast(d2v, __builtin_amdgcn_raw_buffer_load_b128(r, off + 16 * k, 0, 0));
        v[2 * k] = a.x; v[2 * k + 1] = a.y;
    }
}
__device__ __forceinline__ void bstore8(Rsrc r, uint32_t off, const double (&v)[8])
{
#pragma unroll
    for (int k = 0; k < 4; k++) {
        d2v a = {v[2 * k], v[2 * k + 1]};
        __builtin_amdgcn_raw_buffer_store_b128(__builtin_bit_cast(u4v, a), r, off + 16 * k, 0, 0);
    }
}
__device__ __forceinline__ void bstore4(Rsrc r, uint32_t off, float a0, float a1, float a2, float a3)
{
    f4v a = {a0, a1, a2, a3};
    __builtin_amdgcn_raw_buffer_store_b128(__builtin_bit_cast(u4v, a), r, off, 0, 0);
}
__device__ __forceinline__ float bload1f(Rsrc r, uint32_t off)
{
    return __builtin_bit_cast(float, __builtin_amdgcn_raw_buffer_load_b32(r, off, 0, 0));
}

__host__ __device__ __forceinline__ int colpos(int lx, int ly)
{
    if (ly == 0) return lx;
    if (ly == 7) return 8 + lx;
    if (lx == 0) return 15 + ly;
    if (lx == 7) return 21 + ly;
    return 28 + (ly - 1) * 6 + (lx - 1);
}
__host__ __device__ __forceinline__ void colpos_inv(int p, int &lx, int &ly)
{
    if (p < 8) { lx = p; ly = 0; }
    else if (p < 16) { lx = p - 8; ly = 7; }
    else if (p < 22) { lx = 0; ly = p - 15; }
    else if (p < 28) { lx = 7; ly = p - 21; }
    else { lx = 1 + (p - 28) % 6; ly = 1 + (p - 28) / 6; }
}

template <typename R> struct Lay {
    static constexpr int ZQ = 128 / (int)sizeof(R);
    static constexpr int BPL = ZQ / 8;
};
template <typename R>
__device__ __forceinline__ uint32_t zoff_bytes(int zb)
{
    constexpr int LB = Lay<R>::BPL == 4 ? 2 : 1, LS = sizeof(R) == 4 ? 5 : 6;
    const uint32_t u = (uint32_t)zb;
    return ((u >> LB) << 13) | ((u & (uint32_t)(Lay<R>::BPL - 1)) << LS);
}
template <typename R>
__device__ __forceinline__ uint32_t tile_bytes(const FsmLaunch &L) { return (uint32_t)L.nzq * 8192u; }

template <typename R>
__device__ __forceinline__ size_t brick_index(const FsmLaunch &L, int x, int y, int z)
{
    constexpr int ZQ = Lay<R>::ZQ;
    const int tile = (y >> 3) * L.ntx + (x >> 3);
    return (((size_t)tile * L.nzq + z / ZQ) * 64 + colpos(x & 7, y & 7)) * ZQ + z % ZQ;
}

template <typename R>
__device__ __forceinline__ float event_time(const FsmLaunch &L, const R *u, int e)
{
    const int node = L.ev_node[e];
    const int nxy = L.nx * L.ny;
    const int z = node / nxy, rem = node - z * nxy, y = rem / L.nx, x = rem - y * L.nx;
    if (!L.ev_frac) return (float)u[brick_index<R>(L, x, y, z)];
    const float wx = L.ev_frac[3 * e], wy = L.ev_frac[3 * e + 1], wz = L.ev_frac[3 * e + 2];
    const int x1 = min(x + 1, L.nx - 1), y1 = min(y + 1, L.ny - 1), z1 = min(z + 1, L.nz - 1);
    float c[8];
#pragma unroll
    for (int k = 0; k < 8; k++)
        c[k] = (float)u[brick_index<R>(L, (k & 1) ? x1 : x, (k & 2) ? y1 : y, (k & 4) ? z1 : z)];
    float a[4];
#pragma unroll
    for (int k = 0; k < 4; k++) a[k] = __fadd_rn(c[2 * k], __fmul_rn(wx, __fsub_rn(c[2 * k + 1], c[2 * k])));
    const float b0 = __fadd_rn(a[0], __fmul_rn(wy, __fsub_rn(a[1], a[0])));
    const float b1 = __fadd_rn(a[2], __fmul_rn(wy, __fsub_rn(a[3], a[2])));
    return __fadd_rn(b0, __fmul_rn(wz, __fsub_rn(b1, b0)));
}

template <typename R>
__device__ __forceinline__ void skip_solve(const FsmLaunch &L, unsigned solve)
{
    const int lane = threadIdx.x;
    if (lane == 0) {
        if (L.solve_clock) {
            const unsigned long long t = __builtin_amdgcn_s_memrealtime();
            L.solve_clock[2 * (size_t)solve] = t;
            L.solve_clock[2 * (size_t)solve + 1] = t;
        }
        if (L.niter) L.niter[solve] = 0;
        if (L.ierr) L.ierr[solve] = 0;
    }
    if (L.ttab)
        for (int e = lane; e < L.nev; e += 64) L.ttab[(size_t)solve * L.nev + e] = FLT_MAX;
}

struct BcBoxes {
    int n;
    int *box;
};

#ifdef MCEIK_TRAFFIC
#define TRAF(S, k, pred, bytes)                                                                         \
    do {                                                                                                \
        const unsigned n_ = (unsigned)__builtin_popcountll(__ballot(pred));                             \
        if (threadIdx.x == 0) (S).scratch[8 + (k)] += (int)(n_ * (unsigned)(bytes));                     \
    } while (0)
#define TRAFU(S, k, bytes)                                                                              \
    do {                                                                                                \
        if (threadIdx.x == 0) (S).scratch[8 + (k)] += (int)(bytes);                                     \
    } while (0)
#endif
#ifdef MCEIK_TRAFFIC
#define TRAF_FLUSH(L, S)                                                                                \
    do {                                                                                                \
        asm volatile("" ::: "memory");                                                                  \
        if (threadIdx.x == 0 && (L).traffic)                                                            \
            for (int k_ = 0; k_ < MCEIK_TRAFFIC_N; k_++) {                                              \
                atomicAdd((L).traffic + k_, (unsigned long long)(unsigned)(S).scratch[8 + k_]);         \
                (S).scratch[8 + k_] = 0;                                                                \
            }                                                                                           \
        asm volatile("" ::: "memory");                                                                  \
    } while (0)
#else
#define TRAF(S, k, pred, bytes) do { } while (0)
#define TRAFU(S, k, bytes) do { } while (0)
#define TRAF_FLUSH(L, S) do { } while (0)
#endif

__device__ __forceinline__ void tile_cells(int t, int n, unsigned magic, int &c0, int &nc)
{
    const int a = t * 8, b = min(t * 8 + 7, n - 1);
    c0 = (int)(((unsigned)a * magic) >> 20);
    nc = (int)(((unsigned)b * magic) >> 20) - c0 + 1;
}
__device__ __forceinline__ void block_zcells(const FsmLaunch &L, int kb, int tz, int &cz0, int &ncz)
{
    const int a = tz * kb * 8, b = min(a + kb * 8, L.nz) - 1;
    cz0 = (int)(((unsigned)a * L.magic_rz) >> 20);
    ncz = (int)(((unsigned)b * L.magic_rz) >> 20) - cz0 + 1;
}

__device__ __forceinline__ void bload4(Rsrc r, uint32_t off, float (&v)[4])
{
    f4v a = __builtin_bit_cast(f4v, __builtin_amdgcn_raw_buffer_load_b128(r, off, 0, 0));
    v[0] = a.x; v[1] = a.y; v[2] = a.z; v[3] = a.w;
}
__device__ __forceinline__ void bload4(Rsrc r, uint32_t off, double (&v)[4])
{
    d2v a = __builtin_bit_cast(d2v, __builtin_amdgcn_raw_buffer_load_b128(r, off, 0, 0));
    d2v b = __builtin_bit_cast(d2v, __builtin_amdgcn_raw_buffer_load_b128(r, off + 16, 0, 0));
    v[0] = a.x; v[1] = a.y; v[2] = b.x; v[3] = b.y;
}
__device__ __forceinline__ void bstore1(Rsrc r, uint32_t off, float v)
{
    __builtin_amdgcn_raw_buffer_store_b32(__builtin_bit_cast(unsigned, v), r, off, 0, 0);
}
__device__ __forceinline__ void bstore1(Rsrc r, uint32_t off, double v)
{
    __builtin_amdgcn_raw_buffer_store_b64(__builtin_bit_cast(u2v, v), r, off, 0, 0);
}
__device__ __forceinline__ float bload1(Rsrc r, uint32_t off, float)
{
    return __builtin_bit_cast(float, __builtin_amdgcn_raw_buffer_load_b32(r, off, 0, 0));
}
__device__ __forceinline__ double bload1(Rsrc r, uint32_t off, double)
{
    return __builtin_bit_cast(double, __builtin_amdgcn_raw_buffer_load_b64(r, off, 0, 0));
}

template <typename R, int SLOWMODE>
__device__ __forceinline__ double slow_at(const FsmLaunch &L, const void *slow_model, int x, int y, int z)
{
    if (SLOWMODE == 0)
        return (double)reinterpret_cast<const R *>(slow_model)[brick_index<R>(L, x, y, z)];
    const float *si = reinterpret_cast<const float *>(slow_model);
    asm volatile("" : "+v"(si));
    return (double)si[((size_t)(z / L.nrz) * L.ncy + y / L.nry) * L.ncx + x / L.nrx];
}

__device__ __forceinline__ int wave_max(int v)
{
#pragma unroll
    for (int o = 32; o > 0; o >>= 1) v = max(v, __shfl_xor(v, o, 64));
    return v;
}

template <bool FAST>
__device__ __forceinline__ float godunov_v(float a, float b, float c, float f, float ff, float ff2, float ff3)
{
    const unsigned ia = __builtin_bit_cast(unsigned, a), ib = __builtin_bit_cast(unsigned, b),
                   ic = __builtin_bit_cast(unsigned, c);
    unsigned u1, u2, u3;
    asm("v_min3_u32 %0, %1, %2, %3" : "=v"(u1) : "v"(ia), "v"(ib), "v"(ic));
    asm("v_med3_u32 %0, %1, %2, %3" : "=v"(u2) : "v"(ia), "v"(ib), "v"(ic));
    asm("v_max3_u32 %0, %1, %2, %3" : "=v"(u3) : "v"(ia), "v"(ib), "v"(ic));
    const float a1 = __builtin_bit_cast(float, u1), a2 = __builtin_bit_cast(float, u2),
                a3 = __builtin_bit_cast(float, u3);
    const float d2 = a2 - a1, d3 = a3 - a1;
    const float e = d3 - d2;
    const float d22 = d2 * d2, d33 = d3 * d3;
    const float t = d33 + e * e;
    const bool two = t >= ff;
    const float r2 = ff2 - d22;
    const float sm = d2 + d3;
    const float disc = ff3 - (d22 + t);
    const float rad = two ? r2 : disc;
    const float s = FAST ? sqrt_normal(rad) : __builtin_sqrtf(rad);
    const float y23 = ((two ? d2 : sm) + s) * (two ? 0.5f : (1.0f / 3.0f));
    const float y = !(f > d2) ? f : y23;
    const unsigned ix = __builtin_bit_cast(unsigned, a1 + y);
    return __builtin_bit_cast(float, __builtin_elementwise_min(ix, 0x7f7fffffu));
}
template <bool FAST>
__device__ __forceinline__ double godunov_v(double a, double b, double c, double f, double, double, double)
{
    return godunov_fast64<FAST>(a, b, c, f);
}

template <typename R, int SLOWMODE>
__device__ __forceinline__ bool init_field(const FsmLaunch &L, R *u, Rsrc ur, const void *slow_model, const double *src,
                           BcBoxes &bc)
{
    const int lane = threadIdx.x;
    const R UN = Num<R>::unan();
    const uint32_t nvec = (uint32_t)(L.field_elems / 8);
    R fill[8];
#pragma unroll
    for (int i = 0; i < 8; i++) fill[i] = UN;
    for (uint32_t i = lane; i < nvec; i += 64) bstore8(ur, i * 8u * (uint32_t)sizeof(R), fill);
    __builtin_amdgcn_s_waitcnt(0);
    __builtin_amdgcn_fence(__ATOMIC_SEQ_CST, "workgroup");
    bc.n = L.nsrc;
    bool ok = true;
    for (int s = 0; s < L.nsrc; s++) {
        const double *sp = src + (size_t)s * 4;
        const double ts = sp[0];
        int loc[3][3];
        const int nn[3] = {L.nx, L.ny, L.nz};
        const double org[3] = {L.x0, L.y0, L.z0};
        for (int a = 0; a < 3; a++) {
            double xs = sp[1 + a], x0 = org[a], dx = L.h;
            int n = nn[a], is;
            if (xs <= x0) is = 1;
            else if (xs >= x0 + (double)(n - 1) * dx) is = n;
            else is = (int)((xs - x0) / dx + 0.5) + 1;
            int np = 0;
            loc[a][0] = loc[a][1] = loc[a][2] = -1;
            double xe = x0 + (double)(is - 1) * dx;
            if (xe > xs) { loc[a][0] = is - 1; loc[a][1] = is; np = 2; }
            else if (xe < xs) { loc[a][0] = is; loc[a][1] = is + 1; np = 2; }
            else {
                loc[a][np++] = is - 1;
                loc[a][np++] = is;
                if (is < n - 1) loc[a][np++] = is + 1;
            }
            for (int i = 0; i < np; i++) if (loc[a][i] < 1 || loc[a][i] > n) ok = false;
            int lo = 1 << 30, hi = -1;
            for (int i = 0; i < np; i++) { lo = min(lo, loc[a][i] - 1); hi = max(hi, loc[a][i] - 1); }
            if (lane == 0) { bc.box[6 * s + 2 * a] = lo; bc.box[6 * s + 2 * a + 1] = hi; }
        }
        if (!ok) { bc.n = s; break; }
        if (lane < 27) {
            int i = lane % 3, j = (lane / 3) % 3, k = lane / 9;
            int ix = loc[0][i], iy = loc[1][j], iz = loc[2][k];
            if (ix != -1 && iy != -1 && iz != -1) {
                double x = L.x0 + (double)(ix - 1) * L.h, y = L.y0 + (double)(iy - 1) * L.h,
                       z = L.z0 + (double)(iz - 1) * L.h;
                double ddx = sp[1] - x, ddy = sp[2] - y, ddz = sp[3] - z;
                double dd = __builtin_sqrt((ddx * ddx + ddy * ddy) + ddz * ddz);
                double sl = slow_at<R, SLOWMODE>(L, slow_model, ix - 1, iy - 1, iz - 1);
                R t = (R)(ts + dd * sl);
                size_t idx = brick_index<R>(L, ix - 1, iy - 1, iz - 1);
                R cur = u[idx];
                u[idx] = (__builtin_fabs(dd) < 1.e-10) ? t : (cur < t ? cur : t);
            }
        }
        __builtin_amdgcn_s_waitcnt(0);
        __builtin_amdgcn_fence(__ATOMIC_SEQ_CST, "workgroup");
    }
    __builtin_amdgcn_fence(__ATOMIC_SEQ_CST, "workgroup");
    return ok;
}

__device__ __forceinline__ int next_solve(const FsmLaunch &L, int &pass)
{
    const int g0 = blockIdx.x & 7;
    while (pass < 8) {
        const int g = (g0 + pass) & 7;
        const int lo = (int)((long long)L.nsolve * g / 8), hi = (int)((long long)L.nsolve * (g + 1) / 8);
        unsigned i = 0;
        if (threadIdx.x == 0) i = atomicAdd(L.counter + 32 * g, 1u);
        i = __builtin_amdgcn_readfirstlane(__shfl(i, 0, 64));
        if ((int)i < hi - lo) return L.solve_order ? L.solve_order[lo + (int)i] : lo + (int)i;
        pass++;
    }
    return -1;
}

__device__ __forceinline__ void build_order(const FsmLaunch &L, int *order)
{
    for (int id = threadIdx.x; id < L.ntiles; id += 64) {
        const int txs = id % L.ntx, tys = id / L.ntx, dg = txs + tys;
        int rank = 0;
        for (int e = 0; e < dg; e++)
            rank += min(e, L.nty - 1) - max(0, e - L.ntx + 1) + 1;
        rank += tys - max(0, dg - L.ntx + 1);
        order[rank] = txs | (tys << 16);
    }
}

struct Pos {
    int vb, sp, zbs, ri;
};
__device__ __forceinline__ void pos_init(Pos &p, int vb, int kb, int nr)
{
    p.vb = vb;
    const int v = vb < 0 ? 0 : vb;
    p.sp = v / kb; p.zbs = v - p.sp * kb;
    p.ri = p.sp % nr;
}
__device__ __forceinline__ void pos_adv(Pos &p, int kb, int nr)
{
    const int z1 = p.zbs + (p.vb >= 0 ? 1 : 0);
    const bool wrap = z1 == kb;
    const int r1 = p.ri + (wrap ? 1 : 0);
    p.zbs = wrap ? 0 : z1;
    p.sp += wrap ? 1 : 0;
    p.ri = r1 == nr ? 0 : r1;
    p.vb++;
}
__device__ __forceinline__ bool pos_valid(const Pos &p, int nstream)
{
    return p.vb >= 0 && p.sp < nstream;
}

enum {
    C_ACT = 1,
    C_U0 = 2,
    C_PART = 4,
    C_00 = 8,
    C_BC = 16,
    C_BLK = 32,
    C_ZH = 64,
    C_XOWN = 128,
    C_YOWN = 256,
    F_VALID = 128, F_FIRST = 256, F_LAST = 512, F_SLOW = 1024, F_ZH = 2048
};
__device__ __forceinline__ int ci_tz(unsigned w) { return (int)((w >> 9) & 0x7f); }
__device__ __forceinline__ int ci_ccb(unsigned w) { return (int)w >> 16; }

struct ColTile {
    int tile;
    uint32_t col;
    int fl, cl;
};
template <typename R>
__device__ __forceinline__ void column_tile(const FsmLaunch &L, const BcBoxes &bc, int entry, int lx, int ly,
                                            int lxs, int lys, int rx, int ry, ColTile &t)
{
    const int tx = entry & 0xfff, ty = (entry >> 12) & 0xfff;
    const int x = tx * 8 + lx, y = ty * 8 + ly;
    const uint32_t st = tile_bytes<R>(L);
    const uint32_t col = (uint32_t)(ty * L.ntx + tx) * st + (uint32_t)colpos(lx, ly) * 128u;
    int m = (x < L.nx && y < L.ny) ? C_ACT : 0;
    if (lxs == 0 || lxs == 7) {
        const int xn = x + (((lxs == 0) != (rx != 0)) ? -1 : 1);
        if (!(xn >= 0 && xn < L.nx)) m |= C_XOWN;
    }
    if (lys == 0 || lys == 7) {
        const int yn = y + (((lys == 0) != (ry != 0)) ? -1 : 1);
        if (!(yn >= 0 && yn < L.ny)) m |= C_YOWN;
    }
    if (tx * 8 + 8 > L.nx || ty * 8 + 8 > L.ny) m |= C_PART;
    if (x == 0 && y == 0) m |= C_00;
    for (int k = 0; k < bc.n; k++) {
        const int *q = bc.box + 6 * k;
        if (x >= q[0] && x <= q[1] && y >= q[2] && y <= q[3]) m |= C_BC;
    }
    int cx0, ncxt, cy0, ncyt;
    tile_cells(tx, L.nx, L.magic_rx, cx0, ncxt);
    tile_cells(ty, L.ny, L.magic_ry, cy0, ncyt);
    const int xc = x < L.nx ? x : L.nx - 1, yc = y < L.ny ? y : L.ny - 1;
    const int cxl = (int)(((unsigned)xc * L.magic_rx) >> 20) - cx0;
    const int cyl = (int)(((unsigned)yc * L.magic_ry) >> 20) - cy0;
    t.tile = entry & 0xffffff;
    t.col = col;
    t.fl = m;
    t.cl = cyl * ncxt + cxl;
}
__device__ __forceinline__ unsigned column_word(const FsmLaunch &L, int kb, const ColTile &t, int tz, int ri,
                                                int u0flag, int zh)
{
    int cz0, nczb;
    block_zcells(L, kb, tz, cz0, nczb);
    const int ccb = ri * L.ccb + t.cl * nczb - cz0;
    const int m = t.fl | C_BLK | (u0flag ? C_U0 : 0) | (zh ? C_ZH : 0);
    return (unsigned)(m | (tz << 9) | (ccb << 16));
}

__device__ __forceinline__ int halo_edge_lane(int j)
{
    return j < 8 ? j * 8 : j < 16 ? (j - 8) * 8 + 7 : j < 24 ? j - 16 : 56 + (j - 24);
}
__device__ __forceinline__ uint32_t halo_delta(const FsmLaunch &L, uint32_t tile_bytes, int j, int he, int rx, int ry)
{
    const int lxs = he & 7, lys = he >> 3;
    const int lx = rx ? 7 - lxs : lxs, ly = ry ? 7 - lys : lys;
    if (j < 16) {
        const int dx = ((j < 8) != (rx != 0)) ? -1 : 1;
        return (uint32_t)(dx * (int)tile_bytes) + (uint32_t)((colpos((lx + dx) & 7, ly) - colpos(lx, ly)) * 128);
    }
    const int dy = ((j < 24) != (ry != 0)) ? -1 : 1;
    return (uint32_t)(dy * L.ntx * (int)tile_bytes) + (uint32_t)((colpos(lx, (ly + dy) & 7) - colpos(lx, ly)) * 128);
}
__device__ __forceinline__ unsigned dpp_swap_pair(unsigned v)
{
    return (unsigned)__builtin_amdgcn_mov_dpp((int)v, 0xB1, 0xf, 0xf, false);
}
template <int CCR>
__device__ __forceinline__ void cc_issue(const FsmLaunch &L, int kb, Rsrc sr, int entry, float (&v)[CCR], int &size)
{
    const int lane = threadIdx.x;
    const int tx = entry & 0xfff, ty = (entry >> 12) & 0xfff, tz = (entry >> 24) & 0xff;
    int cx0, ncxt, cy0, ncyt, cz0, nczb;
    tile_cells(tx, L.nx, L.magic_rx, cx0, ncxt);
    tile_cells(ty, L.ny, L.magic_ry, cy0, ncyt);
    block_zcells(L, kb, tz, cz0, nczb);
    size = entry >= 0 ? ncxt * ncyt * nczb : 0;
    const float rz = __builtin_amdgcn_rcpf((float)nczb), rx = __builtin_amdgcn_rcpf((float)ncxt);
#pragma unroll
    for (int r = 0; r < CCR; r++) {
        const int idx = lane + 64 * r;
        const int t = (int)(((float)idx + 0.5f) * rz), cz = idx - t * nczb;
        const int cyl = (int)(((float)t + 0.5f) * rx), cxl = t - cyl * ncxt;
        const uint32_t off = (uint32_t)((((cz0 + cz) * L.ncy + cy0 + cyl) * L.ncx) + cx0 + cxl) * 4u;
        v[r] = bload1f(sr, idx < size ? off : OOB);
    }
}
template <typename R, int CCR>
__device__ __forceinline__ void cc_write(const FsmLaunch &L, float *cc, int ri, const float (&v)[CCR], int size,
                                         float h)
{
    const int lane = threadIdx.x;
#pragma unroll
    for (int r = 0; r < CCR; r++) {
        const int idx = lane + 64 * r;
        if (idx < size) cc[ri * L.ccb + idx] = sizeof(R) == 4 ? v[r] * h : v[r];
    }
}

struct Stream {
    int cursor, tile, k, k0, wait;
};

}
```

mceik_amd/csrc/fsm_kernel.hip:

```cpp
#include <hip/hip_runtime.h>
#include <float.h>
#include <stdint.h>
#include <stdlib.h>

#include <type_traits>

#include "fsm_common.h"
#include "fsm_device.h"
#include "fsm_hold.h"
#include "fsm_update.h"


namespace {


template <typename R, bool CMP = false>
struct Smem {
    using clk_t = typename std::conditional<CMP, unsigned short, int>::type;
    int *box;
    float *cc;
    int *order;
    clk_t *lastproc, *lastchg;
    int *ring;
    int *scratch;
// ... 555 lines not shown
    for (int pos = 0; pos <= (AH - 1) / kb; pos++) {
        int zh;
        const int e = decide_any(pos, dri, zh);
        if (e == -2) {
            if (pos == 0) return 0;
            nstream = pos;
            break;
        }
        admit<R>(L, kb, S, bc, e, zh, dri, clock0 + pos, clock_it, lx, ly, lxs, lys, rx, ry, ct);
        if (SLOWMODE == 2 && e >= 0) {
            cc_issue<CCR>(L, kb, sr, e, ccv, ccsize);
            TRAFU(S, 5, ccsize * 4);
            cc_write<R, CCR>(L, S.cc, dri, ccv, ccsize, (float)L.h);
        }
        ndecided = pos + 1;
        if (++dri == nr) dri = 0;
    }
    asm volatile("" ::: "memory");
    Pos p3;
    pos_init(p3, -d, kb, nr);
    BInfo b0 = brick_info<R, RZ, ZSH>(L, kb, S, p3, nstream, lx, ly, bc, cinfo_at(L, S, p3.ri, lane, lanecol));
    bload8(ur, b0.seg, c);
    if (SLOWMODE != 2) prefetch_slow<R, SLOWMODE>(L, S, sr, b0, lx, ly, fq);
    Pos pe;
    pos_init(pe, -hd, kb, nr);
    {
        const uint32_t ho = halo_offset<R, RZ>(L, kb, pe, nstream, hh, cinfo_at(L, S, pe.ri, he, hcol), hbit, hdelta);
        bload4(ur, ho, hq);
        TRAF(S, 1, ho != OOB, 4 * sizeof(R));
    }
    zc = bload1(ur, b0.zh, R());
    TRAF(S, 0, b0.seg != OOB, 8 * sizeof(R));
    TRAF(S, 2, b0.zh != OOB, sizeof(R));
    pos_adv(p3, kb, nr);
    BInfo b1 = brick_info<R, RZ, ZSH>(L, kb, S, p3, nstream, lx, ly, bc, cinfo_at(L, S, p3.ri, lane, lanecol));
    bload8(ur, b1.seg, n);
    pos_adv(pe, kb, nr);
    {
        const uint32_t ho = halo_offset<R, RZ>(L, kb, pe, nstream, hh, cinfo_at(L, S, pe.ri, he, hcol), hbit, hdelta);
        bload4(ur, ho, hn);
        TRAF(S, 1, ho != OOB, 4 * sizeof(R));
    }
    zn = bload1(ur, b1.zh, R());
    TRAF(S, 0, b1.seg != OOB, 8 * sizeof(R));
    TRAF(S, 2, b1.zh != OOB, sizeof(R));
#pragma unroll
    for (int i = 0; i < 8; i++) {
        r[i] = UN;
        if (SLOWMODE != 2) S.sf[i * 64 + lane] = fq[i] * hr;
    }
    store4(S.xr + hso, hq);
    store_row(S.xr, 0, lane, r);
    store_row(S.xr, 1, lane, n);
    if (FL64) {
        Pos pn = p3;
        pos_adv(pn, kb, nr);
        const bool nl = pn.vb >= 0 && (pn.zbs & 1) == 1;
        const uint32_t sn = nl ? brick_info<R, RZ, ZSH>(L, kb, S, pn, nstream, lx, ly, bc,
                                                         cinfo_at(L, S, pn.ri, lane, lanecol)).seg
                               : OOB;
        const bool nlp = dpp_swap_pair((unsigned)nl) != 0u;
        const uint32_t snp = dpp_swap_pair(sn);
        const uint32_t s0 = (nl ? sn : (nlp ? snp : OOB)) + (uint32_t)(lane & 1) * 16u;
        d2v x = __builtin_bit_cast(d2v, __builtin_amdgcn_raw_buffer_load_b128(ur, s0, 0, 0));
        d2v y = __builtin_bit_cast(d2v, __builtin_amdgcn_raw_buffer_load_b128(ur, s0 + 32u, 0, 0));
        double *hd = reinterpret_cast<double *>(S.xr) + XHOLD(0) + 2 * lane;
        hd[0] = x.x; hd[1] = x.y; hd[128] = y.x; hd[129] = y.y;
    }
#pragma unroll
    for (int i = 0; i < 4; i++) hq[i] = hn[i];
#pragma unroll
    for (int i = 0; i < 8; i++) asm volatile("" : "+v"(c[i]), "+v"(n[i]));
#pragma unroll
    for (int i = 0; i < 4; i++) asm volatile("" : "+v"(hq[i]));
    asm volatile("" : "+v"(zc), "+v"(zn));
    asm volatile("" ::: "memory");

    int ph = AH % kb;
    int cc_pend = -1;
    int B = 0;
    bool ccfill = false;
    int ccri = 0;
    auto decide_step = [&]() __attribute__((always_inline)) {
        ccfill = false;
        ccri = 0;
        if (ph == 0 && nstream == 0x7fffffff) {
            const int pos = ndecided;
            int zh;
            const int e = decide_any(pos, dri, zh);
            if (e == -2) {
                nstream = pos;
            } else {
                admit<R>(L, kb, S, bc, e, zh, dri, clock0 + pos, clock_it, lx, ly, lxs, lys, rx, ry, ct);
                if (SLOWMODE == 2 && e >= 0) {
                    cc_issue<CCR>(L, kb, sr, e, ccv, ccsize);
                    TRAFU(S, 5, ccsize * 4);
                    ccfill = true;
                    ccri = dri;
                }
                ndecided = pos + 1;
                if (++dri == nr) dri = 0;
            }
        }
    };
    auto more = [&]() __attribute__((always_inline)) -> bool {
        return !(nstream != 0x7fffffff && B >= nstream * kb + 14);
    };
    auto step = [&](R (&c)[8], R (&n)[8], R (&hq)[4], R (&hn)[4]) __attribute__((always_inline)) -> bool {
        pos_adv(p3, kb, nr);
        pos_adv(pe, kb, nr);
        const u2v ci3 = cinfo_at(L, S, p3.ri, lane, lanecol), cie = cinfo_at(L, S, pe.ri, he, hcol);
        __builtin_amdgcn_sched_barrier(0);
        const BInfo b3 = brick_info<R, RZ, ZSH>(L, kb, S, p3, nstream, lx, ly, bc, ci3);
        if (PAIR)
            pair_issue(ur, b3.seg, qa, qb);
        else if (FL64)
            line_issue64(ur, b3.lseg, p3.vb >= 0 && (p3.zbs & 1) == 0, la, lh, rowl, rowo);
        else
            bload8(ur, b3.seg, q);
        zq = __any(b3.zh != OOB) ? bload1(ur, b3.zh, R()) : R(0);
        {
            const uint32_t ho = halo_offset<R, RZ>(L, kb, pe, nstream, hh, cie, hbit, hdelta);
            bload4(ur, ho, hn);
            TRAF(S, 1, ho != OOB, 4 * sizeof(R));
            TRAF(S, 0, b3.seg != OOB, 8 * sizeof(R));
            TRAF(S, 2, b3.zh != OOB, sizeof(R));
        }
        if (SLOWMODE != 2) prefetch_slow<R, SLOWMODE>(L, S, sr, b1, lx, ly, fq);

        __builtin_amdgcn_s_setprio(0);
        bool changed = false, nc = false, c0 = false, c7 = false;
        const bool zdsel = HOLD && b0.zd && !(S.fmask[b0.ri] & HOLD_CONT);
        if (__any(b0.fl & F_SLOW))
            brick_update<R, SLOWMODE, FAST, RZ, ZSH, true>(L, S, b0, c, n, r, zc, lx, ly, rx, ry, changed, nc,
                                                           ierr_last, zdsel, c0, c7);
        else if (!__any(notconv))
            brick_update<R, SLOWMODE, FAST, RZ, ZSH, false>(L, S, b0, c, n, r, zc, lx, ly, rx, ry, changed, nc,
                                                            ierr_last, zdsel, c0, c7);
        else
            brick_update<R, SLOWMODE, FAST, RZ, ZSH, false, CMP, false>(L, S, b0, c, n, r, zc, lx, ly, rx, ry,
                                                                        changed, nc, ierr_last, zdsel, c0, c7);
        const bool val = (b0.fl & F_VALID) != 0;
        changed = changed && val;
        notconv |= nc && val;
        nchg += changed ? 1u : 0u;
        __builtin_amdgcn_s_setprio(2);

        if (SLOWMODE == 2) {
            if (kb >= 2) {
                if (cc_pend >= 0) cc_write<R, CCR>(L, S.cc, cc_pend, ccv, ccsize, (float)L.h);
                cc_pend = ccfill ? ccri : -1;
            } else if (ccfill) {
                cc_write<R, CCR>(L, S.cc, ccri, ccv, ccsize, (float)L.h);
            }
        } else {
#pragma unroll
            for (int i = 0; i < 8; i++) S.sf[i * 64 + lane] = fq[i] * hr;
        }
        store4(S.xr + hso, hq);
        R nn[8];
        if (PAIR) {
            pair_finish(qa, qb, reinterpret_cast<float (&)[8]>(nn));
        } else {
#pragma unroll
            for (int i = 0; i < 8; i++) {
                if (!FL64) nn[i] = q[i];
            }
        }
        auto u0_store = [&]() __attribute__((always_inline)) {
            if (__any(b0.fl & C_U0) && !__any(notconv)) {
                R m = fmin_(fmin_(fmin_(c[0], c[1]), fmin_(c[2], c[3])), fmin_(fmin_(c[4], c[5]), fmin_(c[6], c[7])));
                const bool st0 = m < (R)L.conv_thresh && (b0.fl & C_U0);
                if (__any(st0)) bstore8(u0r, st0 ? b0.seg : OOB, c);
                TRAF(S, 4, st0, 8 * sizeof(R));
            }
        };
        constexpr bool LAZYN = sizeof(R) == 8;
        if (LAZYN) u0_store();
        store_row(S.xr, 0, lane, r);
        if (LAZYN) load_row(S.xr, xrow<R>(1, lane), c);
        if (FL64)
            line_write64(reinterpret_cast<double *>(S.xr), rowl, rowo, la, lh);
        else
            store_row(S.xr, 1, lane, nn);
#pragma unroll
        for (int i = 0; i < 4; i++) hq[i] = hn[i];
        zc = zn; zn = zq;
#pragma unroll
        for (int i = 0; i < 8; i++) {
            if (!FL64) asm volatile("" : "+v"(nn[i]));
        }
        if (FL64) {
#pragma unroll
            for (int i = 0; i < 4; i++) asm volatile("" : "+v"(la[i]), "+v"(lh[i]));
        }
        asm volatile("" : "+v"(hq[0]), "+v"(hq[1]), "+v"(hq[2]), "+v"(hq[3]));
        asm volatile("" : "+v"(zn));
        asm volatile("" ::: "memory");

        if (__any(changed)) {
            if (PAIR)
                pair_store(ur, b0.seg, changed, reinterpret_cast<const float (&)[8]>(r));
            else
                bstore8(ur, changed ? b0.seg : OOB, r);
            TRAF(S, 3, changed, 8 * sizeof(R));
        }
        if (!LAZYN) u0_store();
        if constexpr (HOLD) {
            const int zr = (b0.zb8 >> 3) % kb;
            const bool zlo = changed && zr == 0 && c0, zhi = changed && zr == kb - 1 && c7;
            if (changed) atomicOr(&S.fmask[b0.ri], xyface | (zlo ? HOLD_ZLO : 0u) | (zhi ? HOLD_ZHI : 0u));
        } else if (changed) {
            S.lastchg[b0.bid] = (typename Smem<R, CMP>::clk_t)(clock0 + b0.clk);
        }
        asm volatile("" ::: "memory");
        if (!LAZYN) {
#pragma unroll
            for (int i = 0; i < 8; i++) {
                c[i] = n[i];
                n[i] = nn[i];
            }
        }
        b0 = b1;
        b1 = b3;
        if (++ph == kb) ph = 0;
        B++;
        decide_step();
        return more();
    };
    decide_step();
    if (more()) {
        do {
        } while (step(c, n, hq, hn));
    }
    __builtin_amdgcn_s_setprio(0);
    nsteps += (unsigned)B;
    if constexpr (HOLD) {
        const HoldLds<int> H = hold_lds(S);
        for (int q = max(0, nstream - L.infl + 1); q < nstream; q++) hold_settle(L, H, q % nr, clock0 + q);
    }
    return nstream;
}

template <typename R, bool CMP>
__device__ __forceinline__ void verify_small(const FsmLaunch &L, Rsrc ur, Rsrc u0r, const Smem<R, CMP> &S, int clock_it, bool &notconv)
{
    const int lane = threadIdx.x, lx = lane & 7, ly = lane >> 3;
    const R T = (R)L.conv_thresh, tolr = (R)L.tol;
    for (int base = 0; base < L.nblocks; base += 64) {
        const int k = base + lane;
        const bool flag = k < L.nblocks && (CMP ? ((S.cbits[k >> 5] >> (k & 31)) & 1u) != 0
                                                 : S.lastchg[k] >= clock_it);
        unsigned long long m = __ballot(flag);
        while (m) {
            const int bid = base + __builtin_ctzll(m);
            m &= m - 1;
            const int tz = bid / L.ntiles, id = bid - tz * L.ntiles;
            const int tx = id % L.ntx, ty = id / L.ntx;
            const int x = tx * 8 + lx, y = ty * 8 + ly;
            const int zend = min(tz * L.kb + L.kb, L.nzb);
            for (int zb = tz * L.kb; zb < zend; zb++) {
                const uint32_t seg = (uint32_t)id * tile_bytes<R>(L) + zoff_bytes<R>(zb) + (uint32_t)colpos(lx, ly) * 128u;
                R u[8], v0[8];
                bload8(ur, seg, u);
                bload8(u0r, seg, v0);
                TRAF(S, 6, x < L.nx && y < L.ny, 16 * sizeof(R));
#pragma unroll
                for (int i = 0; i < 8; i++) {
                    R dl = v0[i] - u[i];
                    dl = dl < (R)0 ? -dl : dl;
                    if (x < L.nx && y < L.ny && zb * 8 + i < L.nz && u[i] < T && !(dl < tolr)) notconv = true;
                }
            }
            if (__any(notconv)) return;
        }
    }
}

#define FSM_WPE __attribute__((amdgpu_waves_per_eu(sizeof(R) == 8 ? 2 : 1)))
template <typename R, int SLOWMODE, bool FAST, int ZSH, int CCR, int KB>
__global__ __launch_bounds__(64) FSM_WPE void fsm_solve_kernel(FsmLaunch L)
{
    extern __shared__ __attribute__((aligned(16))) unsigned char smem[];
    constexpr bool CMP = sizeof(R) == 8 && KB > 0;
    const Smem<R, CMP> S = smem_bind<R, KB == MCEIK_KB && sizeof(R) == 4 && SLOWMODE == 2, CMP>(L, smem);
    const int lane = threadIdx.x;
    const uint32_t fbytes = (uint32_t)(L.field_elems * sizeof(R));
    build_order(L, S.order);
    int pass = 0;
    for (;;) {
        const int snext = next_solve(L, pass);
        if (snext < 0) break;
        const unsigned solve = (unsigned)snext;
        if (L.solve_clock && lane == 0) L.solve_clock[2 * (size_t)solve] = __builtin_amdgcn_s_memrealtime();
        const int model = (int)solve / L.nstat, station = (int)solve - model * L.nstat;
        if (L.skip && L.skip[(L.model_phase && SLOWMODE != 0 ? L.model_phase[model] : fsm_plain_phase(L, model)) *
                                 L.nstat + station]) {
            skip_solve<R>(L, solve);
            __builtin_amdgcn_s_waitcnt(0);
            __builtin_amdgcn_fence(__ATOMIC_SEQ_CST, "workgroup");
            continue;
        }
        const size_t slot = L.slot_per_solve ? solve : blockIdx.x;
        R *u = reinterpret_cast<R *>(L.u) + slot * L.field_elems;
        R *u0 = reinterpret_cast<R *>(L.u0) + (size_t)blockIdx.x * L.field_elems;
        const void *slow_model;
        uint32_t slow_bytes;
        if (SLOWMODE == 0) {
            slow_model = reinterpret_cast<const R *>(L.slow) + (size_t)model * L.field_elems;
            slow_bytes = fbytes;
        } else {
            const size_t ncell = (size_t)L.ncx * L.ncy * L.ncz;
            slow_model = reinterpret_cast<const float *>(L.slow) + fsm_slow_entry(L, model) * ncell;
            slow_bytes = (uint32_t)(ncell * 4);
        }
        const Rsrc ur = make_rsrc(u, fbytes), u0r = make_rsrc(u0, fbytes), sr = make_rsrc(slow_model, slow_bytes);
        constexpr bool HOLD = CMP;
        if (!HOLD) {
            for (int t = lane; t < L.nblocks; t += 64) {
                S.lastproc[t] = -2; S.lastchg[t] = -3;
            }
        }
        if (lane == 0) { S.scratch[0] = 0; S.scratch[1] = 0; S.scratch[2] = 0; S.scratch[3] = 0; }
#ifdef MCEIK_TRAFFIC
        if (lane == 0)
            for (int k = 0; k < MCEIK_TRAFFIC_N; k++) S.scratch[8 + k] = 0;
#endif
        unsigned nchg = 0, nsteps = 0;
        BcBoxes bc;
        bc.box = S.box;
        const bool ok = init_field<R, SLOWMODE>(L, u, ur, slow_model, L.src + (size_t)station * L.nsrc * 4, bc);
        if constexpr (HOLD) {
            hold_solve_start(L, hold_lds(S), bc, L.nr);
        } else if (lane == 0) {
            for (int k = 0; k < bc.n; k++) {
                const int *q = bc.box + 6 * k;
                for (int tz = q[4] / (8 * L.kb); tz <= q[5] / (8 * L.kb); tz++)
                    for (int ty = q[2] >> 3; ty <= q[3] >> 3; ty++)
                        for (int tx = q[0] >> 3; tx <= q[1] >> 3; tx++)
                            S.lastchg[(tz * L.nty + ty) * L.ntx + tx] = -1;
            }
        }
        asm volatile("" ::: "memory");
        int iters = 0, ierr_last = 0, clock = 64;
        if (ok) {
            int sweeps_left = L.max_sweeps < 0 ? 0x7fffffff : L.max_sweeps;
            for (int it = 0; it < L.maxit && sweeps_left > 0; it++) {
                bool notconv = false;
                if constexpr (HOLD) {
                    hold_iter_start(L, hold_lds(S));
                    clock = 64;
                }
                const int clock_it = clock;
                for (int sw = 0; sw < 8 && sweeps_left > 0; sw++, sweeps_left--) {
                    const int rx = sw & 1, ry = (sw >> 1) & 1;
#ifdef MCEIK_STEPSTATS
                    const int clock_sw = clock;
#endif
                    if (sw & 4)
                        clock += L.infl + sweep<R, SLOWMODE, FAST, true, ZSH, CCR, KB>(
                                              L, ur, u0r, sr, bc, S, rx, ry, clock_it, clock, notconv, ierr_last, nchg,
                                              nsteps);
                    else
                        clock += L.infl + sweep<R, SLOWMODE, FAST, false, ZSH, CCR, KB>(
                                              L, ur, u0r, sr, bc, S, rx, ry, clock_it, clock, notconv, ierr_last, nchg,
                                              nsteps);
#ifdef MCEIK_STEPSTATS
                    {
                        const int c1 = clock - L.infl;
                        unsigned nu = 0;
                        for (int t = lane; t < L.nblocks; t += 64) {
                            const int lp = S.lastproc[t];
                            nu += (lp >= c1 - 0x100000 && lp > 63 && lp >= clock_sw && S.lastchg[t] < lp) ? 1u : 0u;
                        }
                        for (int o = 32; o > 0; o >>= 1) nu += __shfl_xor(nu, o, 64);
                        if (lane == 0) S.scratch[3] += nu;
                    }
#endif
                    __builtin_amdgcn_s_waitcnt(0);
                    __builtin_amdgcn_fence(__ATOMIC_SEQ_CST, "workgroup");
                    TRAF_FLUSH(L, S);
                }
                iters = it + 1;
                if (sweeps_left > 0 || L.max_sweeps < 0) {
                    if (!__any(notconv)) verify_small<R>(L, ur, u0r, S, clock_it, notconv);
                    if (!__any(notconv)) break;
                }
            }
        }
        int ierr = ierr_last;
        for (int o = 32; o > 0; o >>= 1) ierr = max(ierr, __shfl_xor(ierr, o, 64));
        if (!ok) ierr = 1;
        if (L.visit_stats) {
            for (int o = 32; o > 0; o >>= 1) nchg += __shfl_xor(nchg, o, 64);
            asm volatile("" ::: "memory");
            if (lane == 0) {
                atomicAdd(L.visit_stats, (unsigned long long)(unsigned)S.scratch[0]);
#ifdef MCEIK_STEPSTATS
                atomicAdd(L.visit_stats + 1, (unsigned long long)(unsigned)S.scratch[2]);
                atomicAdd(L.visit_stats + 2, (unsigned long long)(unsigned)S.scratch[3]);
#else
                atomicAdd(L.visit_stats + 1, (unsigned long long)(unsigned)S.scratch[1]);
                atomicAdd(L.visit_stats + 2, (unsigned long long)nchg);
                atomicAdd(L.visit_stats + 3, (unsigned long long)nsteps);
#endif
            }
        }
        if (lane == 0) {
            if (L.solve_clock) L.solve_clock[2 * (size_t)solve + 1] = __builtin_amdgcn_s_memrealtime();
            if (L.iter_total) atomicAdd(L.iter_total, (unsigned long long)iters);
            if (L.solve_count) atomicAdd(L.solve_count, 1ull);
            if (L.niter) L.niter[solve] = iters;
            if (L.ierr) L.ierr[solve] = ierr;
        }
        TRAFU(S, 7, (unsigned)(L.field_elems * sizeof(R)) + (L.ttab ? (unsigned)L.nev * (4u + 64u) : 0u));
        TRAF_FLUSH(L, S);
        if (L.ttab) {
            for (int e = lane; e < L.nev; e += 64) L.ttab[(size_t)solve * L.nev + e] = event_time<R>(L, u, e);
        }
        __builtin_amdgcn_s_waitcnt(0);
        __builtin_amdgcn_fence(__ATOMIC_SEQ_CST, "workgroup");
    }
}

template <typename RS, typename RD>
__global__ void to_brick_kernel(const RS *src, RD *dst, FsmLaunch L, int nfield)
{
    size_t n = L.field_elems * (size_t)nfield;
    for (size_t i = blockIdx.x * (size_t)blockDim.x + threadIdx.x; i < n; i += (size_t)gridDim.x * blockDim.x) {
        size_t fld = i / L.field_elems, e = i - fld * L.field_elems;
        constexpr int ZQ = Lay<RD>::ZQ;
        const int zi = (int)(e % ZQ);
        size_t t = e / ZQ;
        const int col = (int)(t & 63); t >>= 6;
        const int zq = (int)(t % L.nzq); const int tile = (int)(t / L.nzq);
        int ty = tile / L.ntx, tx = tile - ty * L.ntx;
        int clx, cly;
        colpos_inv(col, clx, cly);
        int x = tx * 8 + clx, y = ty * 8 + cly, z = zq * ZQ + zi;
        RD v = 0;
        if (x < L.nx && y < L.ny && z < L.nz)
            v = (RD)src[fld * (size_t)L.nx * L.ny * L.nz + ((size_t)z * L.ny + y) * L.nx + x];
        dst[i] = v;
    }
}

template <typename RS, typename RD>
__global__ void from_brick_kernel(const RS *src, RD *dst, FsmLaunch L, int nfield)
{
    size_t nn = (size_t)L.nx * L.ny * L.nz, n = nn * nfield;
    for (size_t i = blockIdx.x * (size_t)blockDim.x + threadIdx.x; i < n; i += (size_t)gridDim.x * blockDim.x) {
        size_t fld = i / nn, e = i - fld * nn;
        int x = (int)(e % L.nx); size_t t = e / L.nx;
        int y = (int)(t % L.ny); int z = (int)(t / L.ny);
        dst[i] = (RD)src[fld * L.field_elems + brick_index<RS>(L, x, y, z)];
    }
}

}

template <typename R, int SLOWMODE, bool FAST, int ZSH, int CCR, int KB>
static hipError_t launch_fsm(const FsmLaunch &L, int nwaves, hipStream_t st)
{
    size_t lds = fsm_lds_bytes(L, sizeof(R));
    if (KB == MCEIK_KB && sizeof(R) == 4 && SLOWMODE == 2 && !fsm_fixed_layout(L, 4)) return hipErrorInvalidValue;
    hipLaunchKernelGGL((fsm_solve_kernel<R, SLOWMODE, FAST, ZSH, CCR, KB>), dim3(nwaves), dim3(64), lds, st, L);
    return hipGetLastError();
}

template <typename R, int SLOWMODE, bool FAST, int ZSH, int CCR, int KB>
static int occupancy_of(size_t lds)
{
    int nb = 0;
    return hipOccupancyMaxActiveBlocksPerMultiprocessor(&nb, fsm_solve_kernel<R, SLOWMODE, FAST, ZSH, CCR, KB>, 64,
                                                        lds) == hipSuccess ? nb : 1;
}

static int variant(const FsmLaunch &L, int is_double)
{
    const int mode = L.slow_mode == 0 ? 0 : (L.cell_cache ? 2 : 1);
    if (is_double) {
        const int v = 9 + mode * 2 + (mode == 2 && L.nrz == 4 && L.ccb <= 64 ? (fsm_compact_layout(L, 8) ? 2 : 1) : 0);
        return v == 15 && L.fast_sqrt ? 16 : v;
    }
    if (mode != 2) return mode * 2;
    return 4 + (L.fast_sqrt ? 1 : 0) + (L.nrz == 4 && L.fast_sqrt && L.ccb <= 64 ? (L.kb == MCEIK_KB ? 3 : 2) : 0);
}

#define FSM_VARIANTS(X)                         \
    X(0, float, 0, false, -1, 1, 0)             \
    X(2, float, 1, false, -1, 1, 0)             \
    X(4, float, 2, false, -1, 4, 0)             \
    X(5, float, 2, true, -1, 4, 0)              \
    X(7, float, 2, true, 2, 1, 0)               \
    X(8, float, 2, true, 2, 1, MCEIK_KB)        \
    X(9, double, 0, false, -1, 1, 0)            \
    X(11, double, 1, false, -1, 1, 0)           \
    X(13, double, 2, false, -1, 4, 0)           \
    X(14, double, 2, false, 2, 1, 0)            \
    X(15, double, 2, false, 2, 1, MCEIK_KB)     \
    X(16, double, 2, true, 2, 1, MCEIK_KB)

hipError_t fsm16_launch(const FsmLaunch &L, int nwaves, hipStream_t st);
int fsm16_occupancy(const FsmLaunch &L);
static bool use_fsm16(const FsmLaunch &L, int is_double)
{
    static const bool on = [] { const char *e = getenv("MCEIK_FSM16"); return !(e && e[0] == '0'); }();
    const int v = variant(L, is_double);
    return on && L.step_z != 8 && (v == 5 || v == 7 || v == 8) && fsm16_eligible(L, 4);
}
size_t fsm_launch_lds_bytes(const FsmLaunch &L, int is_double)
{
    return use_fsm16(L, is_double) ? fsm16_lds_bytes(L) : fsm_lds_bytes(L, is_double ? 8 : 4);
}
int fsm_launch_kind(const FsmLaunch &L, int is_double) { return use_fsm16(L, is_double) ? 16 : 8; }
const char *fsm_launch_name(const FsmLaunch &L, int is_double)
{
    if (use_fsm16(L, is_double))
        return fsm16_fixed_layout(L) ? "fsm16_solve_kernel<2, 1>" : L.ccb <= 64 ? "fsm16_solve_kernel<0, 1>"
                                                                                 : "fsm16_solve_kernel<0, 4>";
    switch (variant(L, is_double)) {
    case 0: return "fsm_solve_kernel<float, 0, false, -1, 1, 0>";
    case 2: return "fsm_solve_kernel<float, 1, false, -1, 1, 0>";
    case 4: return "fsm_solve_kernel<float, 2, false, -1, 4, 0>";
    case 5: return "fsm_solve_kernel<float, 2, true, -1, 4, 0>";
    case 7: return "fsm_solve_kernel<float, 2, true, 2, 1, 0>";
    case 8: return "fsm_solve_kernel<float, 2, true, 2, 1, 4>";
    case 9: return "fsm_solve_kernel<double, 0, false, -1, 1, 0>";
    case 11: return "fsm_solve_kernel<double, 1, false, -1, 1, 0>";
    case 13: return "fsm_solve_kernel<double, 2, false, -1, 4, 0>";
    case 14: return "fsm_solve_kernel<double, 2, false, 2, 1, 0>";
    case 15: return "fsm_solve_kernel<double, 2, false, 2, 1, 4>";
    case 16: return "fsm_solve_kernel<double, 2, true, 2, 1, 4>";
    }
    return "?";
}

__global__ void fsm_zero_words_kernel(unsigned *p, int n)
{
    for (int i = threadIdx.x; i < n; i += blockDim.x) p[i] = 0u;
}
hipError_t fsm_zero_words(unsigned *p, int n, hipStream_t st)
{
    hipLaunchKernelGGL(fsm_zero_words_kernel, dim3(1), dim3(256), 0, st, p, n);
    return hipGetLastError();
}

hipError_t fsm_launch(const FsmLaunch &L, int is_double, int nwaves, hipStream_t st)
{
    if (use_fsm16(L, is_double)) return fsm16_launch(L, nwaves, st);
    switch (variant(L, is_double)) {
#define X(v, R, M, F, Z, CR, K) case v: return launch_fsm<R, M, F, Z, CR, K>(L, nwaves, st);
        FSM_VARIANTS(X)
#undef X
    default: return hipErrorInvalidValue;
    }
}

int fsm_occupancy(const FsmLaunch &L, int is_double)
{
    if (use_fsm16(L, is_double)) return fsm16_occupancy(L);
    const size_t lds = fsm_lds_bytes(L, is_double ? 8 : 4);
    switch (variant(L, is_double)) {
#define X(v, R, M, F, Z, CR, K) case v: return occupancy_of<R, M, F, Z, CR, K>(lds);
        FSM_VARIANTS(X)
#undef X
    default: return 1;
    }
}

hipError_t fsm_to_brick_f64(const double *src, void *dst, int dst_double, const FsmLaunch &L, int nfield, hipStream_t st)
{
    if (dst_double) hipLaunchKernelGGL((to_brick_kernel<double, double>), dim3(1024), dim3(256), 0, st, src, (double *)dst, L, nfield);
    else hipLaunchKernelGGL((to_brick_kernel<double, float>), dim3(1024), dim3(256), 0, st, src, (float *)dst, L, nfield);
    return hipGetLastError();
}

hipError_t fsm_from_brick_f64(const void *src, int src_double, double *dst, const FsmLaunch &L, int nfield, hipStream_t st)
{
    if (src_double) hipLaunchKernelGGL((from_brick_kernel<double, double>), dim3(1024), dim3(256), 0, st, (const double *)src, dst, L, nfield);
    else hipLaunchKernelGGL((from_brick_kernel<float, double>), dim3(1024), dim3(256), 0, st, (const float *)src, dst, L, nfield);
    return hipGetLastError();
}

hipError_t fsm_from_brick_f32(const float *src, float *dst, const FsmLaunch &L, int nfield, hipStream_t st)
{
    hipLaunchKernelGGL((from_brick_kernel<float, float>), dim3(1024), dim3(256), 0, st, src, dst, L, nfield);
    return hipGetLastError();
}

hipError_t fsm_to_brick_f32(const float *src, float *dst, const FsmLaunch &L, int nfield, hipStream_t st)
{
    hipLaunchKernelGGL((to_brick_kernel<float, float>), dim3(1024), dim3(256), 0, st, src, dst, L, nfield);
    return hipGetLastError();
}
```

Baseline: 635.2.

## Lazily initialize travel-time field blocks on first touch instead of full fill

```diff
diff --git a/mceik_amd/csrc/capi.hip b/mceik_amd/csrc/capi.hip
--- a/mceik_amd/csrc/capi.hip
+++ b/mceik_amd/csrc/capi.hip
@@ -118,6 +118,8 @@
     L.max_waves = b->max_waves;
     L.traffic = b->traffic;
     L.step_z = b->step_z;
+    L.u_stride = L.field_elems +
+                 (fsm_launch_kind(L, is_double) == 16 && fsm16_fixed_layout(L) ? FSM16_UNAN_LINE / 4 : 0);
 }
 
 static int g_device_cus = 0;
@@ -196,7 +198,7 @@
     w.nwaves = batch_waves(L, is_double);
     const size_t zfw = fsm_launch_kind(L, is_double) == 16 ? zf_bytes(L, es) : 0;
     {
-        const size_t per_wave = 2 * L.field_elems * es + zfw;
+        const size_t per_wave = (L.u_stride + L.field_elems) * es + zfw;
         const long cap = (long)(ws_budget_bytes() / (per_wave ? per_wave : 1));
         if (cap >= 1 && w.nwaves > cap) w.nwaves = (int)cap;
     }
@@ -205,7 +207,7 @@
     size_t slow_bytes = b->slow_mode == 0 ? (size_t)b->nmodel * L.field_elems * es : 0;
     w.u = w.slow + ((slow_bytes + 255) & ~(size_t)255);
     size_t nu = b->u_out ? (size_t)L.nsolve : (size_t)w.nwaves;
-    w.u0 = w.u + nu * L.field_elems * es;
+    w.u0 = w.u + nu * L.u_stride * es;
     w.zf = w.u0 + (size_t)w.nwaves * L.field_elems * es;
     w.total = w.zf + (size_t)w.nwaves * zfw;
     return w;
diff --git a/mceik_amd/csrc/fsm16_kernel.hip b/mceik_amd/csrc/fsm16_kernel.hip
--- a/mceik_amd/csrc/fsm16_kernel.hip
+++ b/mceik_amd/csrc/fsm16_kernel.hip
@@ -45,6 +45,7 @@
     unsigned *meta;
     unsigned char *fz;
     unsigned *vbits, *cbits;
+    unsigned *tbits;
 };
 template <bool FIXED>
 __device__ __forceinline__ Smem16 smem16_bind(const FsmLaunch &L, unsigned char *base)
@@ -55,7 +56,7 @@
         off[3] = F16_LASTPROC; off[4] = F16_LASTCHG; off[2] = F16_ORDER;
         off[9] = F16_ORDER + mceik_align16((size_t)L.ntiles * 2);
         off[10] = off[9] + mceik_align16((size_t)L.ntiles);
-        off[0] = off[10] + f16_bitmap_bytes(L);
+        off[0] = off[10] + f16_bitmap_bytes(L, true);
     } else {
         fsm16_smem_layout(L, off);
     }
@@ -73,6 +74,7 @@
     S.fz = base + off[9];
     S.vbits = reinterpret_cast<unsigned *>(base + off[10]);
     S.cbits = S.vbits + (L.nblocks + 31) / 32;
+    S.tbits = S.cbits + (L.nblocks + 31) / 32;
     S.scratch = reinterpret_cast<int *>(base + off[6]);
     S.xr = reinterpret_cast<float *>(base + off[7]);
     S.meta = reinterpret_cast<unsigned *>(base + off[8]);
@@ -281,6 +283,16 @@
 
 #define LW_G(p) (9 + 5 * (p))
 #define LW_CCB 19
+#define LW_XUN (1u << 29)
+#define LW_YUN (1u << 30)
+#define LW_FIRST (1u << 31)
+#define W1_FT (1u << 25)
+static_assert((C_XOWN << 22) == LW_XUN && (C_YOWN << 22) == LW_YUN, "halo_src");
+__device__ __forceinline__ uint32_t unan_line(const FsmLaunch &L) { return (uint32_t)L.field_elems * 4u; }
+__device__ __forceinline__ uint32_t seg_first(const FsmLaunch &L, uint32_t seg, unsigned w)
+{
+    return (w & LW_FIRST) && seg != OOB ? unan_line(L) + (seg & 64u) : seg;
+}
 template <bool RZ>
 __device__ __forceinline__ unsigned lean_word(const FsmLaunch &L, const Fsm16Geo &g, const ColTile &ct, int tz, int ri,
                                               int u0flag, int zh)
@@ -312,9 +324,11 @@
     const unsigned gp = (w >> (ph ? LW_G(1) : LW_G(0))) & 31u;
     const bool pv = pos_valid(p, nstream);
     const bool valid = pv && (gp & 16u);
-    const uint32_t off = base + ((uint32_t)(ph ^ (RZ ? 1 : 0)) << 6);
+    const uint32_t hb = (uint32_t)(ph ^ (RZ ? 1 : 0)) << 6;
+    const uint32_t off = base + hb;
+    const bool ft = (w & LW_FIRST) != 0;
     b.seg = valid ? off : OOB;
-    b.lseg = pv && (w & ((16u << LW_G(0)) | (16u << LW_G(1)))) ? off : OOB;
+    b.lseg = pv && (w & ((16u << LW_G(0)) | (16u << LW_G(1)))) ? (ft ? unan_line(L) : base) + hb : OOB;
     b.zh = valid && (gp & 8u) ? off + (RZ ? 8192u - 64u : 124u - 8192u) : OOB;
     const bool zd = valid && ph == 1 && !(gp & 2u);
     if (b.zh != OOB) b.zh = zf_boundary<float, RZ>(L, S.ring_b[p.ri], false, lx, ly);
@@ -337,27 +351,32 @@
         }
         if (bcm) fl |= F_SLOW;
     }
-    const int ccb = (int)(w >> LW_CCB) + (RZ ? -4 * ph : 4 * ph);
-    b.w1 = (uint32_t)fl | ((uint32_t)ph << 12) | ((uint32_t)p.ri << 20) | (zd ? W1_ZD : 0u);
+    const int ccb = (int)((w >> LW_CCB) & 0x3ffu) + (RZ ? -4 * ph : 4 * ph);
+    b.w1 = (uint32_t)fl | ((uint32_t)ph << 12) | ((uint32_t)p.ri << 20) | (zd ? W1_ZD : 0u) | (ft ? W1_FT : 0u);
     b.w2 = ((uint32_t)ccb & 0xffffu) | ((uint32_t)p.sp << 16);
     b.w3 = ((uint32_t)S.ring_b[p.ri] & 0xffffu) | (bcm << 16);
     return b;
 }
+__device__ __forceinline__ uint32_t halo_src(const FsmLaunch &L, unsigned me, uint32_t base, unsigned hbit,
+                                             uint32_t hdelta)
+{
+    return (me & (hbit << 22)) ? unan_line(L) : base + ((me & hbit) ? 0u : hdelta);
+}
 template <bool RZ>
-__device__ __forceinline__ uint32_t halo_offset_lean(const Pos &pe, int nstream, int half, unsigned me, uint32_t base,
-                                                     unsigned hbit, uint32_t hdelta)
+__device__ __forceinline__ uint32_t halo_offset_lean(const FsmLaunch &L, const Pos &pe, int nstream, int half,
+                                                     unsigned me, uint32_t base, unsigned hbit, uint32_t hdelta)
 {
     const int ph = pe.zbs;
     const bool valid = pos_valid(pe, nstream) && ((me >> (ph ? LW_G(1) : LW_G(0))) & 16u);
-    const uint32_t o = base + ((me & hbit) ? 0u : hdelta) + ((uint32_t)(ph ^ (RZ ? 1 : 0)) << 6) + (uint32_t)half * 32u;
+    const uint32_t o = halo_src(L, me, base, hbit, hdelta) + ((uint32_t)(ph ^ (RZ ? 1 : 0)) << 6) + (uint32_t)half * 32u;
     return valid ? o : OOB;
 }
 template <bool RZ>
-__device__ __forceinline__ uint32_t halo_line_lean(const Pos &pe, int nstream, unsigned me, uint32_t base,
-                                                   unsigned hbit, uint32_t hdelta)
+__device__ __forceinline__ uint32_t halo_line_lean(const FsmLaunch &L, const Pos &pe, int nstream, unsigned me,
+                                                   uint32_t base, unsigned hbit, uint32_t hdelta)
 {
     const bool valid = pos_valid(pe, nstream) && (me & ((16u << LW_G(0)) | (16u << LW_G(1))));
-    return valid ? base + ((me & hbit) ? 0u : hdelta) : OOB;
+    return valid ? halo_src(L, me, base, hbit, hdelta) : OOB;
 }
 __device__ __forceinline__ unsigned dpp_swap_quad_half(unsigned v)
 {
@@ -372,10 +391,11 @@
     return brick_info16<RZ>(L, g, kb, S, p, nstream, lx, ly, bc, meta, col);
 }
 template <bool RZ, bool LEAN>
-__device__ __forceinline__ uint32_t halo_offset_any(const Fsm16Geo &g, int kb, const Pos &pe, int nstream, int half,
-                                                    unsigned meta, uint32_t col, unsigned hbit, uint32_t hdelta)
-{
-    if (LEAN) return halo_offset_lean<RZ>(pe, nstream, half, meta, col, hbit, hdelta);
+__device__ __forceinline__ uint32_t halo_offset_any(const FsmLaunch &L, const Fsm16Geo &g, int kb, const Pos &pe,
+                                                    int nstream, int half, unsigned meta, uint32_t col, unsigned hbit,
+                                                    uint32_t hdelta)
+{
+    if (LEAN) return halo_offset_lean<RZ>(L, pe, nstream, half, meta, col, hbit, hdelta);
     return halo_offset16<RZ>(g, kb, pe, nstream, half, meta, col, hbit, hdelta);
 }
 
@@ -406,7 +426,7 @@
                                         int entry, int zh, int u0flag, int ri, int C, int lx, int ly, int lxs,
                                         int lys, int rx, int ry, ColTile &ct)
 {
-    unsigned meta = 0;
+    unsigned meta = 0, tw = 0;
     int bid = 0, nbv = 0;
     uint32_t base = 0;
     if (entry >= 0) {
@@ -416,6 +436,15 @@
         if ((entry & 0xffffff) != ct.tile) column_tile<float>(L, bc, entry, lx, ly, lxs, lys, rx, ry, ct);
         meta = LEAN ? lean_word<RZ>(L, g, ct, tz, ri, u0flag, zh) : column_word(L, L.kb, ct, tz, ri, u0flag, zh);
         base = (uint32_t)(ty * L.ntx + tx) * tile_bytes<float>(L) + (LEAN ? (uint32_t)tz << 13 : 0u);
+        if (LEAN) {
+            const bool xe = (lxs == 0 || lxs == 7) && !(ct.fl & C_XOWN), ye = (lys == 0 || lys == 7) && !(ct.fl & C_YOWN);
+            const int bx = xe ? bid + (((lxs == 0) != (rx != 0)) ? -1 : 1) : bid;
+            const int by = ye ? bid + (((lys == 0) != (ry != 0)) ? -L.ntx : L.ntx) : bid;
+            const unsigned t0 = S.tbits[bid >> 5], t1 = S.tbits[bx >> 5], t2 = S.tbits[by >> 5];
+            tw = t0 | (1u << (bid & 31));
+            meta |= (((t0 >> (bid & 31)) & 1u) ? 0u : LW_FIRST) | (((t1 >> (bx & 31)) & 1u) ? 0u : LW_XUN) |
+                    (((t2 >> (by & 31)) & 1u) ? 0u : LW_YUN);
+        }
     }
     const int nact = L.visit_stats && entry >= 0 ? __builtin_popcountll(__ballot(ct.fl & C_ACT)) : 0;
     asm volatile("" ::: "memory");
@@ -424,6 +453,7 @@
         if (entry >= 0) {
             S.lastproc[bid] = (unsigned short)C;
             S.vbits[bid >> 5] |= 1u << (bid & 31);
+            if (LEAN) S.tbits[bid >> 5] = tw;
             if (L.visit_stats) {
                 S.scratch[0] += nbv;
                 S.scratch[1] += nbv * nact;
@@ -596,18 +626,18 @@
     asm volatile("" ::: "memory");
     Pos p3, pe;
     pos_init(p3, -d, kb, nr);
-    BInfo16 b0 = brick_info_any<RZ, LEAN>(L, g, kb, S, p3, nstream, lx, ly, bc, S.meta[p3.ri * 64 + lane],
-                                  S.ring_base[p3.ri] + lanecol);
+    unsigned mw = S.meta[p3.ri * 64 + lane];
+    BInfo16 b0 = brick_info_any<RZ, LEAN>(L, g, kb, S, p3, nstream, lx, ly, bc, mw, S.ring_base[p3.ri] + lanecol);
     const int pbr = pair_row(0, lane), pbn = pair_row(1, lane);
     {
         float t[16];
-        seg_issue(ur, b0.seg, t);
+        seg_issue(ur, LEAN ? seg_first(L, b0.seg, mw) : b0.seg, t);
         raw_write(S.xr, pbn, t);
         load_row16(S.xr, 1, lane, v);
     }
     pos_init(pe, -hd, kb, nr);
     {
-        const uint32_t ho = halo_offset_any<RZ, LEAN>(g, kb, pe, nstream, hh, S.meta[pe.ri * 64 + he],
+        const uint32_t ho = halo_offset_any<RZ, LEAN>(L, g, kb, pe, nstream, hh, S.meta[pe.ri * 64 + he],
                                               S.ring_base[pe.ri] + hcol, hbit, hdelta);
         bload4h(ur, ho, *reinterpret_cast<float (*)[4]>(&hq[0]));
         bload4h(ur, ho + 16u, *reinterpret_cast<float (*)[4]>(&hq[4]));
@@ -617,19 +647,20 @@
     TRAF(S, 0, b0.seg != OOB, 64);
     TRAF(S, 2, b0.zh != OOB, 4);
     pos_adv(p3, kb, nr);
-    BInfo16 b1 = brick_info_any<RZ, LEAN>(L, g, kb, S, p3, nstream, lx, ly, bc, S.meta[p3.ri * 64 + lane],
-                                  S.ring_base[p3.ri] + lanecol);
+    mw = S.meta[p3.ri * 64 + lane];
+    BInfo16 b1 = brick_info_any<RZ, LEAN>(L, g, kb, S, p3, nstream, lx, ly, bc, mw, S.ring_base[p3.ri] + lanecol);
     {
         float t[16];
-        seg_issue(ur, b1.seg, t);
+        seg_issue(ur, LEAN ? seg_first(L, b1.seg, mw) : b1.seg, t);
         raw_write(S.xr, pbn, t);
     }
     if (FL) {
         Pos pn = p3;
         pos_adv(pn, kb, nr);
         const bool nl = pn.vb >= 0 && pn.zbs == 1;
-        const uint32_t sn = nl ? brick_info_any<RZ, LEAN>(L, g, kb, S, pn, nstream, lx, ly, bc, S.meta[pn.ri * 64 + lane],
-                                                  S.ring_base[pn.ri] + lanecol).seg
+        mw = S.meta[pn.ri * 64 + lane];
+        const uint32_t sn = nl ? seg_first(L, brick_info_any<RZ, LEAN>(L, g, kb, S, pn, nstream, lx, ly, bc, mw,
+                                                                       S.ring_base[pn.ri] + lanecol).seg, mw)
                                : OOB;
         const bool nlp = dpp_swap_pair((unsigned)nl) != 0u;
         const uint32_t snp = dpp_swap_pair(sn);
@@ -644,7 +675,7 @@
     }
     pos_adv(pe, kb, nr);
     if (HFL) {
-        const uint32_t lo = halo_line_lean<RZ>(pe, nstream, S.meta[pe.ri * 64 + he], S.ring_base[pe.ri] + hcol, hbit,
+        const uint32_t lo = halo_line_lean<RZ>(L, pe, nstream, S.meta[pe.ri * 64 + he], S.ring_base[pe.ri] + hcol, hbit,
                                                hdelta);
         const uint32_t lp = dpp_swap_quad_half(lo);
         const uint32_t l1 = hcme == (hpi ^ 1) ? lo : lp, l0 = hcme == hpi ? lo : lp;
@@ -654,7 +685,7 @@
         bload4h(ur, l1 + ob, hB[1]);
         TRAF(S, 1, l1 != OOB, 32);
     } else {
-        const uint32_t ho = halo_offset_any<RZ, LEAN>(g, kb, pe, nstream, hh, S.meta[pe.ri * 64 + he],
+        const uint32_t ho = halo_offset_any<RZ, LEAN>(L, g, kb, pe, nstream, hh, S.meta[pe.ri * 64 + he],
                                               S.ring_base[pe.ri] + hcol, hbit, hdelta);
         bload4h(ur, ho, *reinterpret_cast<float (*)[4]>(&hn[0]));
         bload4h(ur, ho + 16u, *reinterpret_cast<float (*)[4]>(&hn[4]));
@@ -734,7 +765,7 @@
             seg_issue(ur, b3.seg, qa);
         zq = __any(b3.zh != OOB) ? bload1(zr_, b3.zh, 0.0f) : 0.0f;
         if (HFL) {
-            const uint32_t lo = halo_line_lean<RZ>(pe, nstream, me, ce, hbit, hdelta);
+            const uint32_t lo = halo_line_lean<RZ>(L, pe, nstream, me, ce, hbit, hdelta);
             const uint32_t lp = dpp_swap_quad_half(lo);
             const uint32_t sl = hcme == (hpi ^ P) ? lo : lp;
             const uint32_t qo = 16u * (uint32_t)hr;
@@ -746,7 +777,7 @@
             TRAF(S, 0, b3.seg != OOB, 64);
             TRAF(S, 2, b3.zh != OOB, 4);
         } else {
-            const uint32_t ho = halo_offset_any<RZ, LEAN>(g, kb, pe, nstream, hh, me, ce, hbit, hdelta);
+            const uint32_t ho = halo_offset_any<RZ, LEAN>(L, g, kb, pe, nstream, hh, me, ce, hbit, hdelta);
             bload4h(ur, ho, *reinterpret_cast<float (*)[4]>(&hnew[0]));
             bload4h(ur, ho + 16u, *reinterpret_cast<float (*)[4]>(&hnew[4]));
             TRAF(S, 1, ho != OOB, 32);
@@ -820,12 +851,13 @@
         asm volatile("" ::: "memory");
         store_row16(S.xr, 0, lane, v);
         zprev = v[RZ ? 0 : 15];
-        if (__any(changed)) {
+        const bool wr = changed || (LEAN && (b0.w1 & W1_FT));
+        if (__any(wr)) {
             float t[16];
             raw_read(S.xr, pbr, t);
-            raw_store(ur, b0.seg, changed, t);
-        }
-        TRAF(S, 3, changed, 64);
+            raw_store(ur, b0.seg, wr, t);
+        }
+        TRAF(S, 3, wr && b0.seg != OOB, 64);
         {
             const int zr = LEAN ? (b0.zb() ^ (RZ ? 1 : 0)) : b0.zb() % kb;
             const bool zlo = changed && zr == 0 && c0, zhi = changed && zr == kb - 1 && c15;
@@ -901,6 +933,29 @@
             }
         }
     }
+}
+
+__device__ __forceinline__ void fill_untouched16(const FsmLaunch &L, Rsrc ur, const Smem16 &S)
+{
+    const int lane = threadIdx.x;
+    float fill[8];
+#pragma unroll
+    for (int i = 0; i < 8; i++) fill[i] = Num<float>::unan();
+    asm volatile("" ::: "memory");
+    for (int base = 0; base < L.nblocks; base += 64) {
+        const int k = base + lane;
+        const bool flag = k < L.nblocks && ((S.tbits[k >> 5] >> (k & 31)) & 1u) == 0;
+        unsigned long long m = __ballot(flag);
+        while (m) {
+            const int bid = base + __builtin_ctzll(m);
+            m &= m - 1;
+            const int tz = bid / L.ntiles, id = bid - tz * L.ntiles;
+            fill_block(ur, (uint32_t)id * tile_bytes<float>(L) + ((uint32_t)tz << 13), fill);
+            TRAFU(S, 7, 8192);
+        }
+    }
+    __builtin_amdgcn_s_waitcnt(0);
+    __builtin_amdgcn_fence(__ATOMIC_SEQ_CST, "workgroup");
 }
 
 struct McQueue {
@@ -1030,6 +1085,7 @@
     const Fsm16Geo g = fsm16_geo(L);
     const int lane = threadIdx.x;
     const uint32_t fbytes = (uint32_t)(L.field_elems * 4);
+    constexpr bool FT = KB16 == 2;
     build_order16(L, S.order);
     int pass = 0;
     McQueue mq;
@@ -1052,7 +1108,7 @@
         if (L.solve_clock && lane == 0) L.solve_clock[2 * (size_t)solve] = __builtin_amdgcn_s_memrealtime();
         const int model = (int)solve / L.nstat, station = (int)solve - model * L.nstat;
         const size_t slot = L.slot_per_solve ? solve : blockIdx.x;
-        float *u = reinterpret_cast<float *>(L.u) + slot * L.field_elems;
+        float *u = reinterpret_cast<float *>(L.u) + slot * L.u_stride;
         float *u0 = reinterpret_cast<float *>(L.u0) + (size_t)blockIdx.x * L.field_elems;
         const size_t ncell = (size_t)L.ncx * L.ncy * L.ncz;
         const int phase = L.model_phase ? (MC ? mcmcd::ldv(L.model_phase + model) : L.model_phase[model])
@@ -1066,7 +1122,7 @@
         }
         const size_t sentry = !L.model_phase ? (size_t)model : (size_t)model * L.nphase + phase;
         const void *slow_model = reinterpret_cast<const float *>(L.slow) + sentry * ncell;
-        const Rsrc ur = make_rsrc(u, fbytes), u0r = make_rsrc(u0, fbytes),
+        const Rsrc ur = make_rsrc(u, fbytes + (FT ? FSM16_UNAN_LINE : 0)), u0r = make_rsrc(u0, fbytes),
                    sr = make_rsrc(slow_model, (uint32_t)(ncell * 4));
         const size_t zfb = zf_bytes(L, 4);
         const Rsrc zfr = make_rsrc(reinterpret_cast<char *>(L.zf) + (size_t)blockIdx.x * zfb, (uint32_t)zfb);
@@ -1078,7 +1134,8 @@
         unsigned nchg = 0, nsteps = 0;
         BcBoxes bc;
         bc.box = S.box;
-        const bool ok = init_field<float, 1>(L, u, ur, slow_model, L.src + (size_t)station * L.nsrc * 4, bc);
+        const bool ok = init_field<float, 1, FT>(L, u, ur, slow_model, L.src + (size_t)station * L.nsrc * 4, bc,
+                                                 S.tbits);
         hold_solve_start(L, hold_lds16(S), bc, g.nr);
         zf_init<float>(L, zfr, u, bc);
         asm volatile("" ::: "memory");
@@ -1108,6 +1165,7 @@
                 }
             }
         }
+        if (FT) fill_untouched16(L, ur, S);
         int ierr = ierr_last;
         for (int o = 32; o > 0; o >>= 1) ierr = max(ierr, __shfl_xor(ierr, o, 64));
         if (!ok) ierr = 1;
@@ -1128,7 +1186,7 @@
             if (L.niter) L.niter[solve] = iters;
             if (L.ierr) L.ierr[solve] = ierr;
         }
-        TRAFU(S, 7, (unsigned)(L.field_elems * 4) + (L.ttab ? (unsigned)L.nev * (4u + 64u) : 0u));
+        TRAFU(S, 7, (FT ? 0u : (unsigned)(L.field_elems * 4)) + (L.ttab ? (unsigned)L.nev * (4u + 64u) : 0u));
         TRAF_FLUSH(L, S);
         if (L.ttab) {
             for (int e = lane; e < L.nev; e += 64) L.ttab[(size_t)solve * L.nev + e] = event_time<float>(L, u, e);
diff --git a/mceik_amd/csrc/fsm_common.h b/mceik_amd/csrc/fsm_common.h
--- a/mceik_amd/csrc/fsm_common.h
+++ b/mceik_amd/csrc/fsm_common.h
@@ -26,6 +26,7 @@
     unsigned magic_rx, magic_ry, magic_rz;
     int nzq;
     size_t field_elems;
+    size_t u_stride;
     void *u;
     void *u0;
     void *zf;
@@ -175,9 +176,10 @@
 {
     return fsm16_eligible(L, 4) && L.kb == 4 && L.ccb <= 32 && fsm16_geo(L).nr == F16_NR;
 }
-static inline __host__ __device__ size_t f16_bitmap_bytes(const FsmLaunch &L)
-{
-    return mceik_align16((size_t)((L.nblocks + 31) / 32) * 4 * 2);
+#define FSM16_UNAN_LINE 128
+static inline __host__ __device__ size_t f16_bitmap_bytes(const FsmLaunch &L, bool fixed)
+{
+    return mceik_align16((size_t)((L.nblocks + 31) / 32) * 4 * (fixed ? 3 : 2));
 }
 static inline __host__ __device__ size_t fsm16_smem_layout(const FsmLaunch &L, size_t *off)
 {
@@ -187,7 +189,7 @@
         off[3] = F16_LASTPROC; off[4] = F16_LASTCHG; off[2] = F16_ORDER;
         off[9] = F16_ORDER + mceik_align16((size_t)L.ntiles * 2);
         off[10] = off[9] + mceik_align16((size_t)L.ntiles);
-        off[0] = off[10] + f16_bitmap_bytes(L);
+        off[0] = off[10] + f16_bitmap_bytes(L, true);
         return off[0] + nbox;
     }
     const Fsm16Geo g = fsm16_geo(L);
@@ -199,7 +201,7 @@
     off[3] = o; o += mceik_align16(nb * 2);
     off[4] = o; o += mceik_align16(nb * 2);
     off[9] = o; o += mceik_align16((size_t)L.ntiles);
-    off[10] = o; o += f16_bitmap_bytes(L);
+    off[10] = o; o += f16_bitmap_bytes(L, false);
     off[5] = o; o += mceik_align16(nr * 16);
     off[6] = o; o += MCEIK_SCRATCH_BYTES;
     off[7] = o; o += 2 * 4 * MCEIK_X16Q * 4;
diff --git a/mceik_amd/csrc/fsm_device.h b/mceik_amd/csrc/fsm_device.h
--- a/mceik_amd/csrc/fsm_device.h
+++ b/mceik_amd/csrc/fsm_device.h
@@ -259,9 +259,16 @@
     return godunov_fast64<FAST>(a, b, c, f);
 }
 
-template <typename R, int SLOWMODE>
+template <typename R>
+__device__ __forceinline__ void fill_block(Rsrc ur, uint32_t base, const R (&fill)[8])
+{
+    const uint32_t o = base + (uint32_t)threadIdx.x * 128u;
+#pragma unroll
+    for (int i = 0; i < 128 / (8 * (int)sizeof(R)); i++) bstore8(ur, o + 8u * (uint32_t)sizeof(R) * i, fill);
+}
+template <typename R, int SLOWMODE, bool FT = false>
 __device__ __forceinline__ bool init_field(const FsmLaunch &L, R *u, Rsrc ur, const void *slow_model, const double *src,
-                           BcBoxes &bc)
+                           BcBoxes &bc, unsigned *tbits = nullptr)
 {
     const int lane = threadIdx.x;
     const R UN = Num<R>::unan();
@@ -269,7 +276,22 @@
     R fill[8];
 #pragma unroll
     for (int i = 0; i < 8; i++) fill[i] = UN;
-    for (uint32_t i = lane; i < nvec; i += 64) bstore8(ur, i * 8u * (uint32_t)sizeof(R), fill);
+    if (FT) {
+        for (int w = lane; w < (L.nblocks + 31) / 32; w += 64) tbits[w] = 0;
+        if (lane < 128 / (8 * (int)sizeof(R)))
+            bstore8(ur, (uint32_t)(L.field_elems * sizeof(R)) + (uint32_t)lane * 8u * (uint32_t)sizeof(R), fill);
+        if (mceik_div_up(L.nz, 16) & 1) {
+            for (int t = 0; t < L.ntiles; t++) {
+                const uint32_t o = (uint32_t)t * tile_bytes<R>(L) + ((uint32_t)(L.nzq - 1) << 13) +
+                                   (uint32_t)lane * 128u + 64u;
+                bstore8(ur, o, fill);
+                bstore8(ur, o + 32u, fill);
+            }
+        }
+        asm volatile("" ::: "memory");
+    } else {
+        for (uint32_t i = lane; i < nvec; i += 64) bstore8(ur, i * 8u * (uint32_t)sizeof(R), fill);
+    }
     __builtin_amdgcn_s_waitcnt(0);
     __builtin_amdgcn_fence(__ATOMIC_SEQ_CST, "workgroup");
     bc.n = L.nsrc;
@@ -277,7 +299,7 @@
     for (int s = 0; s < L.nsrc; s++) {
         const double *sp = src + (size_t)s * 4;
         const double ts = sp[0];
-        int loc[3][3];
+        int loc[3][3], blo[3] = {0, 0, 0}, bhi[3] = {0, 0, 0};
         const int nn[3] = {L.nx, L.ny, L.nz};
         const double org[3] = {L.x0, L.y0, L.z0};
         for (int a = 0; a < 3; a++) {
@@ -300,8 +322,26 @@
             int lo = 1 << 30, hi = -1;
             for (int i = 0; i < np; i++) { lo = min(lo, loc[a][i] - 1); hi = max(hi, loc[a][i] - 1); }
             if (lane == 0) { bc.box[6 * s + 2 * a] = lo; bc.box[6 * s + 2 * a + 1] = hi; }
+            blo[a] = lo; bhi[a] = hi;
         }
         if (!ok) { bc.n = s; break; }
+        if (FT) {
+            for (int tz = blo[2] >> 5; tz <= bhi[2] >> 5; tz++)
+                for (int ty = blo[1] >> 3; ty <= bhi[1] >> 3; ty++)
+                    for (int tx = blo[0] >> 3; tx <= bhi[0] >> 3; tx++) {
+                        const int b = (tz * L.nty + ty) * L.ntx + tx;
+                        asm volatile("" ::: "memory");
+                        const unsigned w = tbits[b >> 5];
+                        asm volatile("" ::: "memory");
+                        if (!((w >> (b & 31)) & 1u)) {
+                            fill_block(ur, (uint32_t)(ty * L.ntx + tx) * tile_bytes<R>(L) + ((uint32_t)tz << 13), fill);
+                            if (lane == 0) tbits[b >> 5] = w | (1u << (b & 31));
+                        }
+                    }
+            asm volatile("" ::: "memory");
+            __builtin_amdgcn_s_waitcnt(0);
+            __builtin_amdgcn_fence(__ATOMIC_SEQ_CST, "workgroup");
+        }
         if (lane < 27) {
             int i = lane % 3, j = (lane / 3) % 3, k = lane / 9;
             int ix = loc[0][i], iy = loc[1][j], iz = loc[2][k];
diff --git a/mceik_amd/csrc/fsm_kernel.hip b/mceik_amd/csrc/fsm_kernel.hip
--- a/mceik_amd/csrc/fsm_kernel.hip
+++ b/mceik_amd/csrc/fsm_kernel.hip
@@ -881,7 +881,7 @@
             continue;
         }
         const size_t slot = L.slot_per_solve ? solve : blockIdx.x;
-        R *u = reinterpret_cast<R *>(L.u) + slot * L.field_elems;
+        R *u = reinterpret_cast<R *>(L.u) + slot * L.u_stride;
         R *u0 = reinterpret_cast<R *>(L.u0) + (size_t)blockIdx.x * L.field_elems;
         const void *slow_model;
         uint32_t slow_bytes;
@@ -1032,7 +1032,7 @@
         size_t fld = i / nn, e = i - fld * nn;
         int x = (int)(e % L.nx); size_t t = e / L.nx;
         int y = (int)(t % L.ny); int z = (int)(t / L.ny);
-        dst[i] = (RD)src[fld * L.field_elems + brick_index<RS>(L, x, y, z)];
+        dst[i] = (RD)src[fld * L.u_stride + brick_index<RS>(L, x, y, z)];
     }
 }
 
```

After: 641.8, median of 6. +1.0%, better.
